# qpc001/ORB_SLAM2_Commit

Measured on AMD Instinct MI355X. Metric: frames/sec ORB extract+match (2k kp) + LocalBA iters/sec, KITTI-00 stereo, higher is better.
Workload: dtype u8; 1 GPU; KITTI-00 stereo 1241x376, 2000 features, extract L+R + ComputeStereoMatches; batch_frames_per_gpu=256, global_batch_frames=256, nlevels=8, parallelism=frame-sharded x1, batches_in_flight=4

## Files before the change

include/orbx_debug.h:

```cpp
#ifndef ORBX_DEBUG_H
#define ORBX_DEBUG_H
#include "orbx.h"
#ifdef __cplusplus
extern "C" {
#endif

enum {
  ORBX_DBG_BLUR_LEVEL = 1,
  ORBX_DBG_CELL_COUNTS = 2,
  ORBX_DBG_CELL_TABLE = 3,
  ORBX_DBG_CANDIDATES = 4,
  ORBX_DBG_OCT_COUNTS = 5,
  ORBX_DBG_OCT_OUT = 6,
  ORBX_DBG_LEVEL_INFO = 7,
  ORBX_DBG_PATCH_SLOTS = 8
};

long long orbx_debug_copy(orbx_extractor* h, int what, int image, int arg, void* dst, size_t cap);

enum {
  ORBX_LP_LEVELS = 1,
  ORBX_LP_RESIZE = 2,
  ORBX_LP_BOUNDS = 3,
  ORBX_LP_GRIDS = 4,
  ORBX_LP_REMAP = 5,
  ORBX_LP_XTAB = 6,
  ORBX_LP_YTAB = 7,
  ORBX_LP_PATH = 8,
  ORBX_LP_FAST = 9,
  ORBX_LP_OCTREE = 10,
  ORBX_LP_CELLS = 11,
  ORBX_LP_OCT_LEVELS = 12,
  ORBX_LP_OCT_PYRAMID = 13
};
long long orbx_debug_launch_plan(const orbx_extractor_params* params, int width, int height, int what, int a0,
                                 int a1, int a2, long long* dst, size_t cap);

orbx_status orbx_debug_stereo_keypoints(orbx_extractor* left, orbx_extractor* right, const orbx_keypoint* kpsL,
                                        const uint8_t* descL, int nL, const orbx_keypoint* kpsR, const uint8_t* descR,
                                        int nR, float bf, float baseline, float* uRight, float* depth, int32_t* sad,
                                        int32_t* nmatches);
int orbx_debug_stereo_keypoints_check(const orbx_keypoint* kps, int n, int nlevels, int width, int height);

orbx_status orbx_debug_octree_candidates(orbx_extractor* h, int n_img, const int32_t* cell_counts,
                                         const uint32_t* candidates, int32_t* oct_count, uint32_t* oct_out);
orbx_status orbx_debug_octree_paths(orbx_extractor* h, int n_img, const int32_t* cell_counts,
                                    const uint32_t* candidates, int depth_cap, int32_t* oct_count,
                                    uint32_t* oct_out, int32_t* paths);
int orbx_debug_octree_candidates_check(const orbx_extractor_params* params, int width, int height, int n_img,
                                       const int32_t* cell_counts, const uint32_t* candidates);

double orbx_debug_atan2_det(double y, double x);

int orbx_debug_lm_step(double state[5], int counts[2], double tempChi, double scale, int ok2, int cube_kind,
                       int ops);

int orbx_debug_exp(const double* x, int n, double* y, int device);
int orbx_debug_sim3_exp(const double update[7], const double S[8], int fix_scale, double out[8], int device);

int orbx_debug_log(const double* x, int n, double* y, int device);
int orbx_debug_acos(const double* x, int n, double* y, int device);
int orbx_debug_sim3_log(const double* S, int n, double* out, int32_t* branch, int device);
int orbx_debug_essgraph_linearize(const orbx_essential_graph_problem* problem, double* meas, double* err,
                                  double* J0, double* J1, double* H, double* b, int device);
int orbx_debug_essgraph_solve(const orbx_essential_graph_problem* problem, const double* H, const double* b,
                              double lambda, double* x, int32_t* ok, int device);
int orbx_debug_essgraph_phases(const orbx_essential_graph_problem* problem, const orbx_essential_graph_result* result,
                               double phase_ms[3], long long* envelope_blocks, int device);

int orbx_debug_ldlt(const double* S, const double* b, int N, double* x, int reps, float* ms);
int orbx_debug_ldlt_ex(const double* S, const double* b, int N, double* x, int reps, float* ms, int kind,
                       unsigned long long* stamps);

#define ORBX_BA_LDLT_AUTO 0
#define ORBX_BA_LDLT_COLUMN 1
#define ORBX_BA_LDLT_BLOCKED 2
#define ORBX_BA_LDLT_TILED 3
typedef struct {
  int ldlt;
  int nan_trial;
  int raise_stop_after;
  int trace;
  int fused_ctl;
} orbx_ba_debug_options;
int orbx_debug_ba_options(orbx_ba* h, const orbx_ba_debug_options* options);

enum {
  ORBX_BA_CAP_HEADER = 0,
  ORBX_BA_CAP_LAMBDA_CHI = 1,
  ORBX_BA_CAP_CQ = 2,
  ORBX_BA_CAP_CT = 3,
  ORBX_BA_CAP_X = 4,
  ORBX_BA_CAP_EERR = 5,
  ORBX_BA_CAP_S = 6,
  ORBX_BA_CAP_BS = 7,
  ORBX_BA_CAP_XP = 8,
  ORBX_BA_CAP_CBAK = 9,
  ORBX_BA_CAP_XBAK = 10,
  ORBX_BA_CAP_XL = 11,
  ORBX_BA_CAP_ACT = 12,
  ORBX_BA_CAP_POSE_CAM = 13,
  ORBX_BA_CAP_PT_ID = 14,
  ORBX_BA_CAP_EROBUST = 15
};
int orbx_debug_ba_capture_select(orbx_ba* h, int phase, int it, int q);
long long orbx_debug_ba_capture_read(orbx_ba* h, int what, void* dst, size_t cap);

int orbx_debug_hbm_copy(void* dst, const void* src, size_t bytes, int reps, float* ms);

int orbx_debug_initializer_host(const float* keys1_xy, int n1, const float K[9], float sigma, int iterations,
                                const float* keys2_xy, int n2, const int32_t* matches12, const int32_t* rand_vals,
                                int n_rand, int* used, float R21[9], float t21[3], float* p3d,
                                uint8_t* triangulated, orbx_initializer_result* result);
float orbx_debug_acosf_det(float x);

typedef struct {
  int raise_after_neighbour;
  int probes;
} orbx_new_points_debug_options;
int orbx_debug_new_points_options(orbx_new_points* h, const orbx_new_points_debug_options* options);
enum {
  ORBX_NP_PROBE_EXIT = 0,
  ORBX_NP_PROBE_COS = 1,
  ORBX_NP_PROBE_F12 = 2,
  ORBX_NP_PROBE_MATCH12 = 3
};
long long orbx_debug_new_points_probe(orbx_new_points* h, int what, void* dst, size_t cap);
int orbx_debug_new_points_host(const orbx_new_points_problem* problem, int neighbour, const int32_t* match12,
                               int32_t* skip, float* baseline, float* median_depth, float F12[9], uint8_t* exit_code,
                               float* cos3, float* pos, float* normal, float* dist);

#ifdef __cplusplus
}
#endif
#endif
```

orb_slam2_commit_amd/_lib.py:

```python
import ctypes as C
import os

import numpy as np

_HERE = os.path.dirname(os.path.abspath(__file__))
LIB_PATH = os.environ.get("ORBX_LIB_OVERRIDE") or os.path.join(_HERE, "liborbx.so")

ORBX_OK = 0
ORBX_ERR_ARG = -1
ORBX_ERR_CAPACITY = -2
ORBX_ERR_HIP = -3
ORBX_ERR_NODEV = -4
ORBX_ERR_SIZE = -5
ORBX_ERR_STATE = -6
ORBX_DEPTH_U16 = 2
ORBX_DEPTH_F32 = 5
_ERRS = {ORBX_ERR_ARG: "bad argument", ORBX_ERR_CAPACITY: "capacity", ORBX_ERR_HIP: "HIP runtime error",
         ORBX_ERR_NODEV: "no HIP device", ORBX_ERR_SIZE: "unsupported geometry", ORBX_ERR_STATE: "no extraction yet"}

KEYPOINT_DTYPE = np.dtype([("x", "<f4"), ("y", "<f4"), ("size", "<f4"), ("angle", "<f4"),
                           ("response", "<f4"), ("octave", "<i4"), ("class_id", "<i4")])
assert KEYPOINT_DTYPE.itemsize == 28


# ... 212 lines not shown
    "orbx_extractor_get_levels": ([P], C.c_int),
    "orbx_extractor_scale_tables": ([P, P, P, P, P], C.c_int),
    "orbx_extractor_tables": ([P, P, P, P], C.c_int),
    "orbx_extractor_set_pyramid_readback": ([P, C.c_int], C.c_int),
    "orbx_extractor_max_keypoints": ([P, C.c_int, C.c_int], C.c_int),
    "orbx_extract": ([P, P, C.c_int, C.c_int, C.c_size_t, P, C.c_int, P, C.POINTER(C.c_int)], C.c_int),
    "orbx_pyramid_level": ([P, C.c_int, C.c_int, P, C.c_size_t, C.POINTER(C.c_int), C.POINTER(C.c_int)], C.c_int),
    "orbx_extract_batch_device": ([P, C.c_int, P, C.c_int, C.c_int, C.c_size_t, P, P, P, C.c_int, P], C.c_int),
    "orbx_stereo_match": ([P, P, P, P, C.c_int, P, P, C.c_int, C.c_float, C.c_float, P, P], C.c_int),
    "orbx_frame_stereo": ([P, P, C.c_size_t, P, C.c_size_t, C.c_int, C.c_int, C.c_float, C.c_float, P, P, C.c_int, P,
                           P, P, C.c_int, P, P, P], C.c_int),
    "orbx_stereo_frames_device": ([P, C.c_int, P, C.c_int, C.c_int, C.c_size_t, P, P, P, C.c_int, C.c_float,
                                   C.c_float, P, P, P, P], C.c_int),
    "orbx_cvt_gray": ([P, C.c_size_t, C.c_size_t, C.c_int, C.c_int, C.c_int, C.c_int, C.c_int, P, C.c_size_t,
                       C.c_size_t, C.c_int], C.c_int),
    "orbx_cvt_gray_device": ([P, P, C.c_size_t, C.c_size_t, C.c_int, C.c_int, C.c_int, C.c_int, C.c_int, P,
                              C.c_size_t, C.c_size_t, P], C.c_int),
    "orbx_frame_rgbd": ([P, P, C.c_size_t, C.c_int, C.c_int, C.c_int, C.c_int, P, C.c_size_t, C.c_int, C.c_int,
                         C.c_int, C.c_float, C.POINTER(Camera), C.c_float, P, P, C.c_int, C.POINTER(C.c_int), P, P,
                         P], C.c_int),
    "orbx_rgbd_frames_device": ([P, C.c_int, P, C.c_int, C.c_int, C.c_int, C.c_int, C.c_size_t, C.c_size_t, P,
                                 C.c_int, C.c_size_t, C.c_size_t, C.c_float, C.POINTER(Camera), C.c_float, P, P, P,
                                 C.c_int, P, P, P, P, P], C.c_int),
    "orbx_descriptor_distance_device": ([P, P, C.c_int, P, P], C.c_int),
    "orbx_search_by_bow_kf_f": ([C.POINTER(BowSide), C.POINTER(BowSide), C.c_float, C.c_int, P,
                                 C.POINTER(C.c_int), C.c_int], C.c_int),
    "orbx_search_by_bow_kf_kf": ([C.POINTER(BowSide), C.POINTER(BowSide), C.c_float, C.c_int, P,
                                  C.POINTER(C.c_int), C.c_int], C.c_int),
    "orbx_search_by_bow_device": ([C.POINTER(BowProblem), C.c_int, P], C.c_int),
    "orbx_pnp_create": ([C.POINTER(PnpProblem), C.POINTER(PnpParams), C.c_int, C.POINTER(C.c_void_p)], C.c_int),
    "orbx_pnp_create_many": ([P, C.c_int, C.POINTER(PnpParams), C.c_int, P], C.c_int),
    "orbx_pnp_create_many_device": ([P, P, P, P, P, C.c_int, C.POINTER(PnpParams), C.c_int, P], C.c_int),
    "orbx_pnp_destroy": ([P], C.c_int),
    "orbx_pnp_get_params": ([P, C.POINTER(C.c_int), C.POINTER(C.c_int), C.POINTER(C.c_float)], C.c_int),
    "orbx_pnp_set_ransac_parameters": ([P, P, C.POINTER(PnpParams)], C.c_int),
    "orbx_pnp_iterate": ([P, C.c_int, P, C.c_int, C.POINTER(C.c_int), C.POINTER(C.c_int), P, P,
                          C.POINTER(C.c_int), C.POINTER(C.c_int)], C.c_int),
    "orbx_pnp_iterate_stream": ([P, C.c_int, C.POINTER(RandState), C.POINTER(C.c_int), P, P, C.POINTER(C.c_int),
                                 C.POINTER(C.c_int)], C.c_int),
    "orbx_voc_load_text": ([C.c_char_p, C.c_size_t, C.c_int, C.POINTER(C.c_void_p)], C.c_int),
    "orbx_voc_destroy": ([P], C.c_int),
    "orbx_voc_info": ([P, P], C.c_int),
    "orbx_voc_transform": ([P, P, P, C.c_int, C.c_int, P, P, P, P, P, P, P], C.c_int),
    "orbx_voc_transform_device": ([P, P, C.c_int, C.c_longlong, P, C.c_int, C.c_int, C.c_int, P, P, P, P, P, P, P, P],
                                  C.c_int),
    "orbx_kfdb_create": ([P, C.c_int, C.POINTER(C.c_void_p)], C.c_int),
    "orbx_kfdb_destroy": ([P], C.c_int),
    "orbx_kfdb_check_bow": ([P, P, C.c_int, C.c_uint32], C.c_int),
    "orbx_kfdb_add": ([P, C.c_int64, P, P, C.c_int], C.c_int),
    "orbx_kfdb_erase": ([P, C.c_int64], C.c_int),
    "orbx_kfdb_clear": ([P], C.c_int),
    "orbx_kfdb_set_neighbours": ([P, P, P, P, C.c_int], C.c_int),
    "orbx_kfdb_reloc_candidates": ([P, C.c_uint64, P, P, C.c_int, P, C.c_int, C.POINTER(C.c_int)], C.c_int),
    "orbx_kfdb_loop_candidates": ([P, C.c_uint64, P, P, C.c_int, P, C.c_int, C.c_float, P, C.c_int,
                                   C.POINTER(C.c_int)], C.c_int),
    "orbx_kfdb_reloc_candidates_device": ([P, C.c_uint64, P, P, P, P, C.c_int, P, P], C.c_int),
    "orbx_kfdb_loop_candidates_device": ([P, C.c_uint64, P, P, P, P, C.c_int, C.c_float, P, C.c_int, P, P],
                                         C.c_int),
    "orbx_kfdb_score": ([P, P, P, C.c_int, P, C.c_int, P], C.c_int),
    "orbx_kfdb_read_state": ([P, P, C.c_int, P, P, P, P, P, P], C.c_int),
    "orbx_kfdb_size": ([P, C.POINTER(C.c_int), C.POINTER(C.c_longlong)], C.c_int),
    "orbx_covis_create": ([C.c_int, C.POINTER(C.c_void_p)], C.c_int),
    "orbx_covis_destroy": ([P], C.c_int),
    "orbx_covis_clear": ([P], C.c_int),
    "orbx_covis_check_row": ([P, P, P, C.c_int], C.c_int),
    "orbx_covis_set_keyframe": ([P, C.c_int64, C.c_int, P, P, P], C.c_int),
    "orbx_covis_erase_keyframe": ([P, C.c_int64], C.c_int),
    "orbx_covis_set_points_bad": ([P, P, C.c_int], C.c_int),
    "orbx_covis_size": ([P, C.POINTER(C.c_int), C.POINTER(C.c_longlong), C.POINTER(C.c_int)], C.c_int),
    "orbx_covis_read_keyframe": ([P, C.c_int64, P, P, P, C.c_int, C.POINTER(C.c_int)], C.c_int),
    "orbx_covis_read_points": ([P, P, C.c_int, P, P], C.c_int),
    "orbx_covis_update_connections": ([P, C.c_int64, C.c_int, P, P, C.c_int, C.POINTER(C.c_int), P, P, C.c_int,
                                       C.POINTER(C.c_int)], C.c_int),
    "orbx_covis_vote": ([P, P, C.c_int, P, P, P, C.c_int, C.POINTER(C.c_int), C.POINTER(C.c_int64),
                         C.POINTER(C.c_int32)], C.c_int),
    "orbx_covis_local_points": ([P, P, C.c_int, P, C.c_int, C.POINTER(C.c_int)], C.c_int),
    "orbx_covis_cull": ([P, P, C.c_int, P, C.c_int, P, P, C.c_int, C.POINTER(C.c_int)], C.c_int),
    "orbx_track_gather_device": ([C.POINTER(TrackGather), C.c_int, P], C.c_int),
    "orbx_frame_points_device": ([C.POINTER(FramePoints), C.c_int, P], C.c_int),
    "orbx_track_step_device": ([C.POINTER(TrackStep), C.c_int, P], C.c_int),
    "orbx_search_by_projection": ([C.POINTER(ProjProblem), C.c_int], C.c_int),
    "orbx_search_by_sim3": ([C.POINTER(Sim3Problem), C.c_int], C.c_int),
    "orbx_search_for_initialization": ([C.POINTER(InitProblem), C.c_int], C.c_int),
    "orbx_search_by_projection_device": ([C.POINTER(ProjProblem), C.c_int, P], C.c_int),
    "orbx_pose_optimization": ([C.POINTER(PoseProblem), C.c_int], C.c_int),
    "orbx_pose_optimization_device": ([C.POINTER(PoseProblem), C.c_int, P], C.c_int),
    "orbx_optimize_sim3": ([C.POINTER(OptSim3Problem), C.c_int], C.c_int),
    "orbx_optimize_sim3_device": ([C.POINTER(OptSim3Problem), C.c_int, P], C.c_int),
    "orbx_optimize_essential_graph": ([C.POINTER(EssGraphProblem), C.POINTER(EssGraphResult), C.c_int], C.c_int),
    "orbx_optimize_essential_graph_device": ([C.POINTER(EssGraphProblem), C.POINTER(EssGraphResult), P], C.c_int),
    "orbx_sim3_from_tcw": ([P, P], None),
    "orbx_search_for_triangulation": ([C.POINTER(TriProblem), C.c_int], C.c_int),
    "orbx_search_for_triangulation_device": ([C.POINTER(TriProblem), C.c_int, P], C.c_int),
    "orbx_new_points_create": ([C.c_int, C.POINTER(C.c_void_p)], C.c_int),
    "orbx_new_points_destroy": ([P], C.c_int),
    "orbx_new_points_stop_flag": ([P, C.POINTER(C.POINTER(C.c_int))], C.c_int),
    "orbx_create_new_map_points": ([P, C.POINTER(NewPointsProblem), C.POINTER(NewPointsResult)], C.c_int),
    "orbx_create_new_map_points_bool": ([P, C.POINTER(NewPointsProblem), C.POINTER(NewPointsResult), P], C.c_int),
    "orbx_create_new_map_points_device": ([P, C.POINTER(NewPointsProblem), C.POINTER(NewPointsResult), P], C.c_int),
    "orbx_distinctive_descriptors": ([P, P, C.c_int, P, P, C.c_int], C.c_int),
    "orbx_distinctive_descriptors_device": ([P, P, C.c_int, P, P, P], C.c_int),
    "orbx_undistort_keypoints": ([P, C.c_int, C.POINTER(Camera), P, C.c_int], C.c_int),
    "orbx_undistort_keypoints_device": ([P, P, C.c_int, C.c_int, P, P, P], C.c_int),
    "orbx_pnp_iterate_candidates": ([P, C.c_int, C.c_int, C.POINTER(RandState), P, P, C.POINTER(C.c_int)], C.c_int),
    "orbx_pnp_iterate_many": ([P, C.c_int, C.c_int, P, P, P], C.c_int),
    "orbx_sim3_create": ([C.POINTER(Sim3SolverProblem), C.POINTER(Sim3Params), C.c_int, C.POINTER(C.c_void_p)],
                         C.c_int),
    "orbx_sim3_create_many": ([P, C.c_int, C.POINTER(Sim3Params), C.c_int, P], C.c_int),
    "orbx_sim3_destroy": ([P], C.c_int),
    "orbx_sim3_set_ransac_parameters": ([P, C.POINTER(Sim3Params)], C.c_int),
    "orbx_sim3_get_params": ([P, C.POINTER(C.c_int), C.POINTER(C.c_int), C.POINTER(C.c_int), C.POINTER(C.c_int)],
                             C.c_int),
    "orbx_sim3_iterate": ([P, C.c_int, P, C.c_int, C.POINTER(C.c_int), C.POINTER(C.c_int), P, P,
                           C.POINTER(C.c_int), C.POINTER(C.c_int)], C.c_int),
    "orbx_sim3_iterate_stream": ([P, C.c_int, C.POINTER(RandState), C.POINTER(C.c_int), P, P, C.POINTER(C.c_int),
                                  C.POINTER(C.c_int)], C.c_int),
    "orbx_sim3_get_estimate": ([P, P, P, C.POINTER(C.c_float)], C.c_int),
    "orbx_sim3_iterate_candidates": ([P, C.c_int, C.c_int, C.POINTER(RandState), P, P, C.POINTER(C.c_int)],
                                     C.c_int),
    "orbx_sim3_iterate_many": ([P, C.c_int, C.c_int, P, P, P], C.c_int),
    "orbx_initializer_create": ([P, C.c_int, P, C.c_float, C.c_int, C.c_int, C.POINTER(C.c_void_p)], C.c_int),
    "orbx_initializer_destroy": ([P], C.c_int),
    "orbx_initializer_initialize": ([P, P, C.c_int, P, P, C.c_int, C.POINTER(C.c_int), P, P, P, P,
                                     C.POINTER(InitializerResult)], C.c_int),
    "orbx_initializer_initialize_stream": ([P, P, C.c_int, P, C.POINTER(RandState), P, P, P, P,
                                            C.POINTER(InitializerResult)], C.c_int),
    "orbx_rand_seed":([C.POINTER(RandState), C.c_uint32], None),
    "orbx_rand_next": ([C.POINTER(RandState)], C.c_int32),
    "orbx_ba_create": ([C.c_int, C.POINTER(C.c_void_p)], C.c_int),
    "orbx_ba_create_priority": ([C.c_int, C.c_int, C.POINTER(C.c_void_p)], C.c_int),
    "orbx_ba_create_masked": ([C.c_int, C.c_void_p, C.c_int, C.POINTER(C.c_void_p)], C.c_int),
    "orbx_stream_create": ([C.c_int, C.c_void_p, C.c_int, C.POINTER(C.c_void_p)], C.c_int),
    "orbx_stream_destroy": ([C.c_void_p], None),
    "orbx_ba_destroy": ([P], C.c_int),
    "orbx_ba_run": ([P, C.POINTER(BaProblem), C.POINTER(BaResult), P], C.c_int),
    "orbx_ba_run_bool": ([P, C.POINTER(BaProblem), C.POINTER(BaResult), P], C.c_int),
    "orbx_ba_run_global": ([P, C.POINTER(BaProblem), C.c_int, C.c_int, C.POINTER(BaResult), P, P], C.c_int),
    "orbx_ba_run_global_bool": ([P, C.POINTER(BaProblem), C.c_int, C.c_int, C.POINTER(BaResult), P, P], C.c_int),
    "orbx_ba_stop_flag":([P, C.POINTER(C.POINTER(C.c_int))], C.c_int),
    "orbx_ba_run_many": ([P, C.c_int, C.POINTER(BaProblem), C.POINTER(BaResult), P], C.c_int),
    "orbx_local_ba": ([C.POINTER(BaProblem), C.POINTER(BaResult), P, C.c_int], C.c_int),
    "orbx_device_count": ([], C.c_int),
    "orbx_version": ([], C.c_char_p),
    "orbx_sizeof": ([C.c_char_p], C.c_longlong),
    "orbx_profile_enable": ([P, C.c_int], C.c_int),
    "orbx_profile_reset": ([P], C.c_int),
    "orbx_profile_read": ([P, C.c_int, C.POINTER(C.c_double), C.POINTER(C.c_longlong),
                           C.POINTER(C.c_char_p)], C.c_int),
    "orbx_debug_copy": ([P, C.c_int, C.c_int, C.c_int, P, C.c_size_t], C.c_longlong),
    "orbx_debug_launch_plan": ([C.POINTER(ExtractorParams), C.c_int, C.c_int, C.c_int, C.c_int, C.c_int, C.c_int, P,
                                C.c_size_t], C.c_longlong),
    "orbx_debug_stereo_keypoints": ([P, P, P, P, C.c_int, P, P, C.c_int, C.c_float, C.c_float, P, P, P, P], C.c_int),
    "orbx_debug_stereo_keypoints_check": ([P, C.c_int, C.c_int, C.c_int, C.c_int], C.c_int),
    "orbx_debug_octree_candidates": ([P, C.c_int, P, P, P, P], C.c_int),
    "orbx_debug_octree_paths": ([P, C.c_int, P, P, C.c_int, P, P, P], C.c_int),    "orbx_debug_octree_candidates_check": ([C.POINTER(ExtractorParams), C.c_int, C.c_int, C.c_int, P, P], C.c_int),
    "orbx_debug_atan2_det": ([C.c_double, C.c_double], C.c_double),
    "orbx_debug_exp": ([P, C.c_int, P, C.c_int], C.c_int),
    "orbx_debug_initializer_host": ([P, C.c_int, P, C.c_float, C.c_int, P, C.c_int, P, P, C.c_int,
                                     C.POINTER(C.c_int), P, P, P, P, C.POINTER(InitializerResult)], C.c_int),
    "orbx_debug_acosf_det": ([C.c_float], C.c_float),
    "orbx_debug_lm_step": ([P, P, C.c_double, C.c_double, C.c_int, C.c_int, C.c_int], C.c_int),
    "orbx_debug_sim3_exp": ([P, P, C.c_int, P, C.c_int], C.c_int),
    "orbx_debug_log": ([P, C.c_int, P, C.c_int], C.c_int),
    "orbx_debug_acos": ([P, C.c_int, P, C.c_int], C.c_int),
    "orbx_debug_sim3_log": ([P, C.c_int, P, P, C.c_int], C.c_int),
    "orbx_debug_essgraph_linearize": ([C.POINTER(EssGraphProblem), P, P, P, P, P, P, C.c_int], C.c_int),
    "orbx_debug_essgraph_solve": ([C.POINTER(EssGraphProblem), P, P, C.c_double, P, P, C.c_int], C.c_int),
    "orbx_debug_essgraph_phases": ([C.POINTER(EssGraphProblem), C.POINTER(EssGraphResult), P, P, C.c_int], C.c_int),
    "orbx_debug_ldlt": ([P, P, C.c_int, P, C.c_int, C.POINTER(C.c_float)], C.c_int),
    "orbx_debug_ldlt_ex": ([P, P, C.c_int, P, C.c_int, C.POINTER(C.c_float), C.c_int, P], C.c_int),
    "orbx_debug_ba_options": ([P, C.POINTER(BaDebugOptions)], C.c_int),
    "orbx_debug_ba_capture_select": ([P, C.c_int, C.c_int, C.c_int], C.c_int),
    "orbx_debug_ba_capture_read": ([P, C.c_int, P, C.c_size_t], C.c_longlong),
    "orbx_debug_new_points_options": ([P, C.POINTER(NewPointsDebugOptions)], C.c_int),
    "orbx_debug_new_points_probe": ([P, C.c_int, P, C.c_size_t], C.c_longlong),
    "orbx_debug_new_points_host": ([C.POINTER(NewPointsProblem), C.c_int, P, P, P, P, P, P, P, P, P, P], C.c_int),
    "orbx_debug_hbm_copy": ([P, P, C.c_size_t, C.c_int, C.POINTER(C.c_float)], C.c_int),
}

BA_CAPTURE_ITEMS = {
    "lambda_chi": (1, np.float64, ()), "cq": (2, np.float64, (4,)), "ct": (3, np.float64, (3,)),
    "X": (4, np.float64, (3,)), "eerr": (5, np.float64, (3,)), "S": (6, np.float64, ()), "bs": (7, np.float64, ()),
    "xp": (8, np.float64, ()), "cbak": (9, np.float64, (7,)), "Xbak": (10, np.float64, (3,)),
    "xl": (11, np.float64, (3,)), "act": (12, np.int32, ()), "pose_cam": (13, np.int32, ()),
    "pt_id": (14, np.int32, ()), "erobust": (15, np.int32, ()),
}
BA_CAPTURE_HEADER = ("fired", "phase", "it", "q", "ok", "trial", "nc", "np", "ne", "na", "npa", "nposes")

_lib = None
_NEWER_ENTRIES = {"orbx_debug_octree_paths"}


def lib():
    global _lib
    if _lib is None:
        if not os.path.exists(LIB_PATH):
            raise RuntimeError("liborbx.so not found at %s -- build it first (make -C orb_slam2_commit_amd/csrc)"
                               % LIB_PATH)
        L = C.CDLL(LIB_PATH)
        for name, (args, res) in SIGNATURES.items():
            if name in _NEWER_ENTRIES and os.environ.get("ORBX_LIB_OVERRIDE") and not hasattr(L, name):
                continue
            fn = getattr(L, name)
            fn.argtypes = args
            fn.restype = res
        _lib = L
    return _lib


def check(code, what):
    if code != ORBX_OK:
        raise OrbxError(code, what)


def ptr(a):
    if a is None:
        return None
    if isinstance(a, np.ndarray):
        try:
            return C.c_void_p(C.addressof(C.c_char.from_buffer(a)))
        except (TypeError, ValueError, BufferError):
            return C.c_void_p(a.__array_interface__["data"][0])
    if hasattr(a, "data_ptr"):
        return C.c_void_p(a.data_ptr())
    raise TypeError(type(a))
```

orb_slam2_commit_amd/csrc/capi.hip:

```cpp
#include <hip/hip_runtime.h>

#include <cmath>
#include <new>
#include <string>

#include "orbx_extractor.h"
#include "orbx_rgbd.h"
#include "orbx_undistort.h"

namespace orbx {

orbx_status get_plan(orbx_extractor* h, int W, int H, DevPlan** out) {
  auto key = std::make_pair(W, H);
  auto it = h->plans.find(key);
  if (it != h->plans.end()) {
    *out = it->second.get();
    return ORBX_OK;
  }
  std::unique_ptr<DevPlan> P(new (std::nothrow) DevPlan());
  if (!P) return ORBX_ERR_HIP;
  orbx_status s = build_plan(h->params, h->tables, W, H, *P);
  if (s != ORBX_OK) return s;
  hipError_t e = P->dG.upload(&P->G, 1);
  if (e == hipSuccess) e = P->dcells.upload(P->cells.data(), P->cells.size());
  if (e == hipSuccess) e = P->dtiles.upload(P->tile_level.data(), P->tile_level.size());
  if (e == hipSuccess) e = P->drzb.upload(P->rzb.data(), P->rzb.size());
  if (e == hipSuccess) e = P->dxt.upload(P->xt.data(), P->xt.size());
  if (e == hipSuccess) e = P->dyt.upload(P->yt.data(), P->yt.size());
  if (e != hipSuccess) return ORBX_ERR_HIP;
  build_launch_plan(*P, P->dxt.p, P->dyt.p, P->drzb.p, P->LP);
  size_t mx = octree_group_smem(P->G.og_all);
  for (int g = 0; g < P->G.n_og; g++) mx = std::max(mx, octree_group_smem(P->G.og[g]));
  if (octree_set_smem_limit(mx) != hipSuccess) return ORBX_ERR_HIP;
  *out = P.get();
  h->plans[key] = std::move(P);
  return ORBX_OK;
}

orbx_status ensure_batch(orbx_extractor* h, const Plan& P, int n) {
  const Geometry& G = P.G;
  hipError_t e = hipSuccess;
  auto chk = [&](hipError_t x) { if (x != hipSuccess) e = x; };
  chk(h->pyr.ensure((size_t)G.pyr_bytes * n + 256));
  chk(h->blur.ensure((size_t)G.blur_bytes * n + 256));
  chk(h->cand.ensure((size_t)G.cand_total * n));
  chk(h->kpos.ensure((size_t)G.cand_total * n));
  chk(h->knode.ensure((size_t)G.cand_total * n));
  chk(h->cell_count.ensure((size_t)std::max(G.ncells, 1) * n));
  chk(h->oct.ensure((size_t)G.oct_total * n));
  chk(h->oct_count.ensure((size_t)G.nlevels * n));
  return hip_status(e);
}

BatchPtrs batch_ptrs(orbx_extractor* h, const uint8_t* in, size_t pitch) {
  BatchPtrs B;
  B.in = in;
  B.in_pitch = pitch;
  B.pyr = h->pyr.p;
  B.blur = h->blur.p;
  B.cand = h->cand.p;
  B.cell_count = h->cell_count.p;
  B.kpos = h->kpos.p;
  B.knode = h->knode.p;
  B.oct = h->oct.p;
  B.oct_count = h->oct_count.p;
  return B;
}

orbx_status run_extract(orbx_extractor* h, DevPlan* P, int n, const uint8_t* d_in, size_t pitch, orbx_keypoint* d_kps,
                        uint8_t* d_desc, int32_t* d_counts, int kp_cap, hipStream_t st) {
  if (kp_cap < P->G.max_kps) return ORBX_ERR_CAPACITY;
  orbx_status s = ensure_batch(h, *P, n);
  if (s != ORBX_OK) return s;
  BatchPtrs B = batch_ptrs(h, d_in, pitch);
  hipError_t e = launch_extract_stages(P->G, P->dG.p, P->dcells.p, P->dtiles.p, P->LP, B, n, d_kps, d_desc, d_counts, kp_cap, st,
                                       &h->timer);
  if (e != hipSuccess) return ORBX_ERR_HIP;
  h->last_plan = P;
  h->last_in = d_in;
  h->last_pitch = pitch;
  h->last_n = n;
  h->last_host = false;
  h->hpyr_valid = false;
  return ORBX_OK;
}

orbx_status run_stereo(orbx_extractor* hl, orbx_extractor* hr, int n_frames, const StereoSides& S, int maxL, float bf,
                       float baseline, float* uR, float* depth, long long out_stride, int32_t* nmatches,
                       hipStream_t st) {
  orbx_extractor* h = hl;
  const DevPlan* P = hl->last_plan;
  hipError_t e = hipSuccess;
  auto chk = [&](hipError_t x) { if (x != hipSuccess) e = x; };
  chk(h->rkeys.ensure((size_t)n_frames * kMaxStereoKps));
  chk(h->oct_start.ensure((size_t)n_frames * (kMaxLevelsPlan + 1)));
  chk(h->rxi.ensure((size_t)n_frames * kMaxStereoKps));
  chk(h->rdesc.ensure((size_t)n_frames * kMaxStereoKps * 2));
  chk(h->rtab.ensure((size_t)n_frames * P->G.nlevels * std::max(P->G.height, 1)));
  chk(h->lrange.ensure((size_t)n_frames * std::max(maxL, 1)));
  chk(h->sad.ensure((size_t)n_frames * out_stride));
  if (e != hipSuccess) return ORBX_ERR_HIP;
  StereoArgs A;
  std::memset(&A, 0, sizeof(A));
  A.kpL = S.L.kps;
  A.dL = S.L.desc;
  A.nL = S.L.counts;
  A.kL_stride = S.L.k_stride;
  A.n_stride_L = S.L.n_stride;
  A.l_step = S.L.step;
  A.l_off = S.L.off;
  A.kpR = S.R.kps;
  A.dR = S.R.desc;
  A.nR = S.R.counts;
  A.kR_stride = S.R.k_stride;
  A.n_stride_R = S.R.n_stride;
  A.r_step = S.R.step;
  A.r_off = S.R.off;
  A.BL = batch_ptrs(hl, hl->last_in, hl->last_pitch);
  A.BR = batch_ptrs(hr, hr->last_in, hr->last_pitch);
  A.nlevels = P->G.nlevels;
  A.maxL = maxL;
  for (int l = 0; l < P->G.nlevels; l++) A.inv_scale[l] = hl->tables.inv_scale[l];
  A.bf = bf;
  A.minZ = baseline;
  A.minD = 0.f;
  A.maxD = bf / baseline;
  A.uR = uR;
  A.depth = depth;
  A.sad = h->sad.p;
  A.out_stride = out_stride;
  A.rkeys = h->rkeys.p;
  A.oct_start = h->oct_start.p;
  A.rxi = h->rxi.p;
  A.rdesc = h->rdesc.p;
  A.rtab = h->rtab.p;
  A.lrange = h->lrange.p;
  A.rows = std::max(P->G.height, 1);
  A.nmatches = nmatches;
  return hip_status(launch_stereo(A, P->dG.p, n_frames, maxL, st, &h->timer));
}

}

using namespace orbx;

namespace {

constexpr size_t kInSlack = 4;

uint64_t fingerprint_words(const void* p, size_t nw, uint64_t h) {
  const uint32_t* w = reinterpret_cast<const uint32_t*>(p);
  for (size_t i = 0; i < nw; i++) {
    h = (h ^ w[i]) * 0x9E3779B97F4A7C15ull;
    h ^= h >> 29;
  }
  return h;
}
uint64_t keypoint_fingerprint(const orbx_keypoint* k, const uint8_t* desc, int n) {
  uint64_t h = 1469598103934665603ull ^ (uint64_t)n;
  h = fingerprint_words(k, (size_t)n * (sizeof(orbx_keypoint) / 4), h);
  if (desc) h = fingerprint_words(desc, (size_t)n * 8, h ^ 0xD6E8FEB86659FD93ull);
  return h;
}


}

extern "C" {

const char* orbx_version(void) { return "orbx 0.1.0 (gfx950)"; }

long long orbx_sizeof(const char* type) {
  if (!type) return -1;
  const std::string t(type);
#define ORBX_SIZEOF(T) \
  if (t == #T) return (long long)sizeof(T);
  ORBX_SIZEOF(orbx_keypoint) ORBX_SIZEOF(orbx_extractor_params) ORBX_SIZEOF(orbx_bow_side)
  ORBX_SIZEOF(orbx_bow_problem) ORBX_SIZEOF(orbx_ba_problem) ORBX_SIZEOF(orbx_ba_result)
  ORBX_SIZEOF(orbx_pnp_problem) ORBX_SIZEOF(orbx_pnp_params) ORBX_SIZEOF(orbx_pnp_result)
  ORBX_SIZEOF(orbx_rand_state) ORBX_SIZEOF(orbx_proj_frame) ORBX_SIZEOF(orbx_proj_problem)
  ORBX_SIZEOF(orbx_tri_kf) ORBX_SIZEOF(orbx_tri_problem) ORBX_SIZEOF(orbx_pose_problem)
  ORBX_SIZEOF(orbx_track_gather) ORBX_SIZEOF(orbx_frame_points) ORBX_SIZEOF(orbx_track_step)
  ORBX_SIZEOF(orbx_camera) ORBX_SIZEOF(orbx_sim3_problem) ORBX_SIZEOF(orbx_init_problem)
  ORBX_SIZEOF(orbx_sim3_solver_problem) ORBX_SIZEOF(orbx_sim3_params) ORBX_SIZEOF(orbx_sim3_result)
  ORBX_SIZEOF(orbx_optimize_sim3_problem) ORBX_SIZEOF(orbx_essential_graph_problem)
  ORBX_SIZEOF(orbx_essential_graph_result) ORBX_SIZEOF(orbx_new_points_kf)
  ORBX_SIZEOF(orbx_new_points_problem) ORBX_SIZEOF(orbx_new_points_result)
#undef ORBX_SIZEOF
  return -1;
}

int orbx_device_count(void) {
  int n = 0;
  if (hipGetDeviceCount(&n) != hipSuccess) return 0;
  return n;
}

orbx_status orbx_extractor_create(const orbx_extractor_params* params, int device, orbx_extractor** out) {
  if (!out || !params_ok(params)) return ORBX_ERR_ARG;
  *out = nullptr;
  int n = 0;
  if (hipGetDeviceCount(&n) != hipSuccess || n <= 0) return ORBX_ERR_NODEV;
  if (device < 0 || device >= n) return ORBX_ERR_ARG;
  if (hipSetDevice(device) != hipSuccess) return ORBX_ERR_HIP;
  orbx_extractor* h = new (std::nothrow) orbx_extractor();
  if (!h) return ORBX_ERR_HIP;
  h->params = *params;
  h->device = device;
  h->tables = make_tables(*params);
  int gauss[7];
  gaussian_int_kernel(gauss);
  if (upload_constants(h->tables.umax, gauss) != hipSuccess ||
      hipStreamCreateWithFlags(&h->stream, hipStreamNonBlocking) != hipSuccess) {
    delete h;
    return ORBX_ERR_HIP;
  }
  *out = h;
  return ORBX_OK;
}

void orbx_extractor_destroy(orbx_extractor* h) {
  if (!h) return;
  (void)hipSetDevice(h->device);
  if (h->stream) {
    (void)hipStreamSynchronize(h->stream);
    (void)hipStreamDestroy(h->stream);
  }
  delete h;
}

int orbx_extractor_get_levels(const orbx_extractor* h) { return h ? h->params.nlevels : ORBX_ERR_ARG; }

orbx_status orbx_extractor_scale_tables(const orbx_extractor* h, float* scale, float* inv_scale, float* sigma2,
                                        float* inv_sigma2) {
  if (!h) return ORBX_ERR_ARG;
  const int n = h->params.nlevels;
  for (int i = 0; i < n; i++) {
    if (scale) scale[i] = h->tables.scale[i];
    if (inv_scale) inv_scale[i] = h->tables.inv_scale[i];
    if (sigma2) sigma2[i] = h->tables.sigma2[i];
    if (inv_sigma2) inv_sigma2[i] = h->tables.inv_sigma2[i];
  }
  return ORBX_OK;
}

orbx_status orbx_extractor_tables(const orbx_extractor* h, int* features_per_level, int* umax, int* pattern) {
  if (!h) return ORBX_ERR_ARG;
  static const int8_t kPattern[512 * 2] = {
#include "brief_pattern_31.inc"
  };
  for (int i = 0; i < h->params.nlevels; i++)
    if (features_per_level) features_per_level[i] = h->tables.nfeat[i];
  for (int v = 0; v < 16; v++)
    if (umax) umax[v] = h->tables.umax[v];
  for (int i = 0; i < 1024; i++)
    if (pattern) pattern[i] = kPattern[i];
  return ORBX_OK;
}

orbx_status orbx_extractor_set_pyramid_readback(orbx_extractor* h, int on) {
  if (!h) return ORBX_ERR_ARG;
  h->pyr_readback = on != 0;
  if (!h->pyr_readback) h->hpyr_valid = false;
  return ORBX_OK;
}

int orbx_extractor_max_keypoints(orbx_extractor* h, int width, int height) {
  if (!h) return ORBX_ERR_ARG;
  DevPlan* P = nullptr;
  orbx_status s = get_plan(h, width, height, &P);
  return s == ORBX_OK ? P->G.max_kps : s;
}

orbx_status orbx_extract(orbx_extractor* h, const uint8_t* img, int width, int height, size_t stride,
                         orbx_keypoint* kps, int cap, uint8_t* desc, int* n) {
  if (!h || !n) return ORBX_ERR_ARG;
  *n = 0;
  if (!img || width <= 0 || height <= 0) return ORBX_OK;
  if (stride < (size_t)width) return ORBX_ERR_ARG;
  if (hipSetDevice(h->device) != hipSuccess) return ORBX_ERR_HIP;
  DevPlan* P = nullptr;
  orbx_status s = get_plan(h, width, height, &P);
  if (s != ORBX_OK) return s;
  const int kcap = P->G.max_kps;
// ... 463 lines not shown
```

orb_slam2_commit_amd/csrc/debug.hip:

```cpp
#include <hip/hip_runtime.h>

#include <cmath>
#include <vector>

#include "../../include/orbx_debug.h"
#include "orbx_extractor.h"

using namespace orbx;

extern "C" long long orbx_debug_copy(orbx_extractor* h, int what, int image, int arg, void* dst, size_t cap) {
  if (!h) return ORBX_ERR_ARG;
  if (!h->last_plan) return ORBX_ERR_STATE;
  const DevPlan& P = *h->last_plan;
  const Geometry& G = P.G;
  if (image < 0 || image >= h->last_n) return ORBX_ERR_ARG;
  if (hipSetDevice(h->device) != hipSuccess) return ORBX_ERR_HIP;
  if (hipStreamSynchronize(h->stream) != hipSuccess) return ORBX_ERR_HIP;
  std::vector<int> host;
  const void* src = nullptr;
  size_t bytes = 0;
  bool device_src = true;
  switch (what) {
    case ORBX_DBG_BLUR_LEVEL: {
      if (arg < 0 || arg >= G.nlevels) return ORBX_ERR_ARG;
      const LevelGeom& L = G.lv[arg];
      bytes = (size_t)L.w * L.h;
      if (dst && cap >= bytes) {
        if (h->blur.ensure((size_t)G.blur_bytes * h->last_n + 256) != hipSuccess) return ORBX_ERR_HIP;
        const BatchPtrs B = batch_ptrs(h, h->last_in, h->last_pitch);
        if (launch_blur(G, P.dG.p, P.dtiles.p, B, h->last_n, h->stream) != hipSuccess ||
            hipStreamSynchronize(h->stream) != hipSuccess)
          return ORBX_ERR_HIP;
        const uint8_t* b = h->blur.p + (size_t)image * G.blur_bytes + L.boff;
        std::vector<uint8_t> tiles((size_t)L.bstride * ((L.h + 7) & ~7));
        if (hipMemcpy(tiles.data(), b, tiles.size(), hipMemcpyDeviceToHost) != hipSuccess) return ORBX_ERR_HIP;
        uint8_t* o = static_cast<uint8_t*>(dst);
        for (int yy = 0; yy < L.h; yy++)
          for (int xx = 0; xx < L.w; xx++)
            o[(size_t)yy * L.w + xx] = tiles[((size_t)(yy >> 3) * (L.bstride >> 4) + (xx >> 4)) * 128 + (yy & 7) * 16 + (xx & 15)];
      }
      return (long long)bytes;
    }
    case ORBX_DBG_CELL_COUNTS:
      src = h->cell_count.p + (size_t)image * G.ncells;
      bytes = sizeof(int) * G.ncells;
      break;
    case ORBX_DBG_CELL_TABLE: {
      int loff = 0;
      for (const CellInfo& c : P.cells) {
        int v[8] = {c.level, c.x0, c.y0, c.x1, c.y1, loff, c.cap, 0};
        host.insert(host.end(), v, v + 8);
        loff += c.cap;
      }
      device_src = false;
      break;
    }
    case ORBX_DBG_CANDIDATES: {
      std::vector<uint32_t> raw((size_t)G.cand_total);
      if (hipMemcpy(raw.data(), h->cand.p + (size_t)image * G.cand_total, raw.size() * 4, hipMemcpyDeviceToHost) !=
          hipSuccess)
        return ORBX_ERR_HIP;
      std::vector<uint32_t> logical;
      logical.reserve(raw.size());
      for (const CellInfo& c : P.cells)
        for (int q = 0; q < c.cap; q++) logical.push_back(raw[cell_slot(c, q)]);
      static_assert(sizeof(uint32_t) == sizeof(int), "host staging is int words");
      host.resize(logical.size());
      std::memcpy(host.data(), logical.data(), logical.size() * 4);
      device_src = false;
      break;
    }
    case ORBX_DBG_OCT_COUNTS:
      src = h->oct_count.p + (size_t)image * G.nlevels;
      bytes = sizeof(int) * G.nlevels;
      break;
    case ORBX_DBG_OCT_OUT:
      src = h->oct.p + (size_t)image * G.oct_total;
      bytes = sizeof(uint32_t) * G.oct_total;
      break;
    case ORBX_DBG_LEVEL_INFO:
      for (int l = 0; l < G.nlevels; l++) {
        const LevelGeom& L = G.lv[l];
        int v[8] = {L.w, L.h, L.cell_begin, L.cell_end, L.oct_off, L.oct_cap, L.nfeat, L.nIni};
        host.insert(host.end(), v, v + 8);
      }
      device_src = false;
      break;
    case ORBX_DBG_PATCH_SLOTS:
      host.assign(patch_slot_table(), patch_slot_table() + 128);
      device_src = false;
      break;
    default:
      return ORBX_ERR_ARG;
  }
  if (!device_src) {
    bytes = host.size() * sizeof(int);
    if (dst) std::memcpy(dst, host.data(), std::min(bytes, cap));
    return (long long)bytes;
  }
  if (dst && cap) {
    if (hipMemcpy(dst, src, std::min(bytes, cap), hipMemcpyDeviceToHost) != hipSuccess) return ORBX_ERR_HIP;
  }
  return (long long)bytes;
}

extern "C" int orbx_debug_stereo_keypoints_check(const orbx_keypoint* kps, int n, int nlevels, int width,
                                                 int height) {
  if (n < 0 || (n > 0 && !kps) || nlevels < 1 || nlevels > kMaxLevelsPlan || width <= 0 || height <= 0)
    return ORBX_ERR_ARG;
  for (int i = 0; i < n; i++) {
    const orbx_keypoint& k = kps[i];
    if (k.octave < 0 || k.octave >= nlevels) return ORBX_ERR_ARG;
    if (!std::isfinite(k.x) || !std::isfinite(k.y) || std::signbit(k.x) || std::signbit(k.y)) return ORBX_ERR_ARG;
    if (!(k.x < (float)width) || !(k.y < (float)height)) return ORBX_ERR_ARG;
  }
  return ORBX_OK;
}

extern "C" orbx_status orbx_debug_stereo_keypoints(orbx_extractor* left, orbx_extractor* right,
                                                   const orbx_keypoint* kpsL, const uint8_t* descL, int nL,
                                                   const orbx_keypoint* kpsR, const uint8_t* descR, int nR, float bf,
                                                   float baseline, float* uRight, float* depth, int32_t* sad,
                                                   int32_t* nmatches) {
  if (!uRight || !depth || !sad || !nmatches || nL < 0 || nR < 0) return ORBX_ERR_ARG;
  if ((nL > 0 && (!kpsL || !descL)) || (nR > 0 && (!kpsR || !descR))) return ORBX_ERR_ARG;
  if (nR > kMaxStereoKps) return ORBX_ERR_CAPACITY;
  if (!left || !right) return ORBX_ERR_ARG;
  if (!left->last_plan || !right->last_plan || !left->last_host || !right->last_host) return ORBX_ERR_STATE;
  const Geometry& G = left->last_plan->G;
  if (G.width != right->last_plan->G.width || G.height != right->last_plan->G.height ||
      G.nlevels != right->last_plan->G.nlevels || left->device != right->device)
    return ORBX_ERR_ARG;
  if (orbx_debug_stereo_keypoints_check(kpsL, nL, G.nlevels, G.width, G.height) != ORBX_OK ||
      orbx_debug_stereo_keypoints_check(kpsR, nR, G.nlevels, G.width, G.height) != ORBX_OK)
    return ORBX_ERR_ARG;
  *nmatches = 0;
  if (nL == 0) return ORBX_OK;
  orbx_extractor* h = left;
  if (hipSetDevice(h->device) != hipSuccess) return ORBX_ERR_HIP;
  BlockCursor cur;
  const size_t o_kL = cur.take<orbx_keypoint>(nL), o_kR = cur.take<orbx_keypoint>(nR),
               o_dL = cur.take<uint8_t>((size_t)nL * 32), o_dR = cur.take<uint8_t>((size_t)nR * 32),
               o_res = cur.take<float>((size_t)2 * nL);
  DevBuf<uint8_t> blk;
  if (blk.ensure(cur.end()) != hipSuccess) return ORBX_ERR_HIP;
  hipError_t e = hipSuccess;
  auto chk = [&](hipError_t x) { if (x != hipSuccess) e = x; };
  hipStream_t st = h->stream;
  const int32_t counts[3] = {nL, nR, 0};
  chk(hipMemcpyAsync(blk.p, counts, sizeof(counts), hipMemcpyHostToDevice, st));
  chk(hipMemcpyAsync(blk.p + o_kL, kpsL, (size_t)nL * sizeof(orbx_keypoint), hipMemcpyHostToDevice, st));
  chk(hipMemcpyAsync(blk.p + o_dL, descL, (size_t)nL * 32, hipMemcpyHostToDevice, st));
  if (nR > 0) {
    chk(hipMemcpyAsync(blk.p + o_kR, kpsR, (size_t)nR * sizeof(orbx_keypoint), hipMemcpyHostToDevice, st));
    chk(hipMemcpyAsync(blk.p + o_dR, descR, (size_t)nR * 32, hipMemcpyHostToDevice, st));
  }
  if (e != hipSuccess) {
    (void)hipStreamSynchronize(st);
    return ORBX_ERR_HIP;
  }
  int32_t* d_counts = (int32_t*)blk.p;
  float* d_ur = (float*)(blk.p + o_res);
  const StereoSides S = StereoSides::handles((const orbx_keypoint*)(blk.p + o_kL), blk.p + o_dL, d_counts,
                                             (const orbx_keypoint*)(blk.p + o_kR), blk.p + o_dR, d_counts + 1);
  orbx_status s = run_stereo(left, right, 1, S, nL, bf, baseline, d_ur, d_ur + nL, nL, d_counts + 2, st);
  if (s == ORBX_OK) {
    chk(hipMemcpyAsync(uRight, d_ur, sizeof(float) * nL, hipMemcpyDeviceToHost, st));
    chk(hipMemcpyAsync(depth, d_ur + nL, sizeof(float) * nL, hipMemcpyDeviceToHost, st));
    chk(hipMemcpyAsync(sad, h->sad.p, sizeof(int32_t) * nL, hipMemcpyDeviceToHost, st));
    chk(hipMemcpyAsync(nmatches, d_counts + 2, sizeof(int32_t), hipMemcpyDeviceToHost, st));
  }
  chk(hipStreamSynchronize(st));
  if (s != ORBX_OK) return s;
  return hip_status(e);
}

constexpr int kOctInjectMaxImages = 64;
static bool octree_candidates_ok(const Plan& P, int n_img, const int32_t* counts, const uint32_t* cand) {
  const Geometry& G = P.G;
  if (n_img < 1 || n_img > kOctInjectMaxImages || !counts || !cand || G.ncells < 1) return false;
  long long total = 0;
  for (const CellInfo& c : P.cells) total += c.cap;
  std::vector<uint8_t> seen;
  for (int img = 0; img < n_img; img++) {
    const int32_t* cnt = counts + (size_t)img * G.ncells;
    const uint32_t* cd = cand + (size_t)img * total;
    for (int l = 0; l < G.nlevels; l++) {
      const LevelGeom& L = G.lv[l];
      seen.assign((size_t)L.w * L.h, 0);
      for (int ci = L.cell_begin; ci < L.cell_end; ci++) {
        if (cnt[ci] < 0 || cnt[ci] > P.cells[ci].cap) return false;
        for (int q = 0; q < cnt[ci]; q++) {
          const uint32_t v = cd[q];
          const int x = (int)(v & 0xFFF), y = (int)((v >> 12) & 0xFFF);
          if (x < L.minBX || x >= L.maxBX || y < L.minBY || y >= L.maxBY) return false;
          uint8_t& s = seen[(size_t)y * L.w + x];
          if (s) return false;
          s = 1;
        }
        cd += P.cells[ci].cap;
      }
    }
  }
  return true;
}

extern "C" int orbx_debug_octree_candidates_check(const orbx_extractor_params* params, int width, int height,
                                                  int n_img, const int32_t* cell_counts, const uint32_t* candidates) {
  if (!params_ok(params) || width <= 0 || height <= 0) return ORBX_ERR_ARG;
  Plan P;
  const orbx_status s = build_plan(*params, make_tables(*params), width, height, P);
  if (s != ORBX_OK) return s;
  return octree_candidates_ok(P, n_img, cell_counts, candidates) ? ORBX_OK : ORBX_ERR_ARG;
}

static orbx_status octree_candidates_run(orbx_extractor* h, int n_img, const int32_t* cell_counts,
                                         const uint32_t* candidates, int32_t* oct_count, uint32_t* oct_out,
                                         int32_t* paths, int depth_cap) {
  if (!h || !oct_count || !oct_out) return ORBX_ERR_ARG;
  if (!h->last_plan) return ORBX_ERR_STATE;
  const DevPlan& P = *h->last_plan;
  const Geometry& G = P.G;
  if (!octree_candidates_ok(P, n_img, cell_counts, candidates)) return ORBX_ERR_ARG;
  if (hipSetDevice(h->device) != hipSuccess) return ORBX_ERR_HIP;
  const size_t n = (size_t)n_img;
  BlockCursor cur;
  const size_t o_cand = cur.take<uint32_t>(n * G.cand_total), o_cnt = cur.take<int>(n * G.ncells),
               o_kpos = cur.take<uint32_t>(n * G.cand_total), o_knode = cur.take<int>(n * G.cand_total),
               o_oct = cur.take<uint32_t>(n * G.oct_total), o_octn = cur.take<int>(n * G.nlevels),
               o_path = cur.take<int>(n * G.nlevels);
  DevBuf<uint8_t> blk;
  if (blk.ensure(cur.end()) != hipSuccess) return ORBX_ERR_HIP;
  std::vector<uint32_t> raw(n * G.cand_total, 0);
  {
    const uint32_t* cd = candidates;
    for (int img = 0; img < n_img; img++)
      for (int ci = 0; ci < G.ncells; ci++) {
        const CellInfo& c = P.cells[ci];
        for (int q = 0; q < cell_counts[(size_t)img * G.ncells + ci]; q++)
          raw[(size_t)img * G.cand_total + cell_slot(c, q)] = cd[q];
        cd += c.cap;
      }
  }
  hipError_t e = hipSuccess;
  auto chk = [&](hipError_t x) { if (x != hipSuccess) e = x; };
  hipStream_t st = h->stream;
  chk(hipMemcpyAsync(blk.p + o_cand, raw.data(), raw.size() * 4, hipMemcpyHostToDevice, st));
  chk(hipMemcpyAsync(blk.p + o_cnt, cell_counts, n * G.ncells * sizeof(int), hipMemcpyHostToDevice, st));
  chk(hipMemsetAsync(blk.p + o_oct, 0xFF, n * G.oct_total * 4, st));
  chk(hipMemsetAsync(blk.p + o_octn, 0xFF, n * G.nlevels * sizeof(int), st));
  chk(hipMemsetAsync(blk.p + o_path, 0xFF, n * G.nlevels * sizeof(int), st));
  if (e == hipSuccess) {
    BatchPtrs B{};
    B.cand = (uint32_t*)(blk.p + o_cand);
    B.cell_count = (int*)(blk.p + o_cnt);
    B.kpos = (uint32_t*)(blk.p + o_kpos);
    B.knode = (int*)(blk.p + o_knode);
    B.oct = (uint32_t*)(blk.p + o_oct);
    B.oct_count = (int*)(blk.p + o_octn);
    size_t mx = octree_group_smem(G.og_all);
    for (int g = 0; g < G.n_og; g++) mx = std::max(mx, octree_group_smem(G.og[g]));
    chk(octree_set_smem_limit(mx));
    if (e == hipSuccess)
      chk(launch_octree(G, P.dG.p, P.dcells.p, B, n_img, st, paths ? (int*)(blk.p + o_path) : nullptr, depth_cap));
  }
  if (e == hipSuccess && paths)
    chk(hipMemcpyAsync(paths, blk.p + o_path, n * G.nlevels * sizeof(int), hipMemcpyDeviceToHost, st));
  if (e == hipSuccess) {
    chk(hipMemcpyAsync(oct_count, blk.p + o_octn, n * G.nlevels * sizeof(int), hipMemcpyDeviceToHost, st));
    chk(hipMemcpyAsync(oct_out, blk.p + o_oct, n * G.oct_total * 4, hipMemcpyDeviceToHost, st));
  }
  chk(hipStreamSynchronize(st));
  return hip_status(e);
}

extern "C" orbx_status orbx_debug_octree_candidates(orbx_extractor* h, int n_img, const int32_t* cell_counts,
                                                    const uint32_t* candidates, int32_t* oct_count,
                                                    uint32_t* oct_out) {
  return octree_candidates_run(h, n_img, cell_counts, candidates, oct_count, oct_out, nullptr, -1);
}

extern "C" orbx_status orbx_debug_octree_paths(orbx_extractor* h, int n_img, const int32_t* cell_counts,
                                               const uint32_t* candidates, int depth_cap, int32_t* oct_count,
                                               uint32_t* oct_out, int32_t* paths) {
  if (!paths || depth_cap < -1) return ORBX_ERR_ARG;
  return octree_candidates_run(h, n_img, cell_counts, candidates, oct_count, oct_out, paths, depth_cap);
}

extern "C" long long orbx_debug_launch_plan(const orbx_extractor_params* params, int width, int height, int what,
                                            int a0, int a1, int a2, long long* dst, size_t cap) {
  std::vector<long long> out;
  auto done = [&]() {
    if (dst) std::memcpy(dst, out.data(), std::min(out.size(), cap) * sizeof(long long));
    return (long long)out.size();
  };
  if (what == ORBX_LP_REMAP) {
    XcdRemap R{};
    if (a0 < 1 || a1 < 1 || a2 < 1 || !make_xcd_remap((unsigned)a0, (unsigned)a1, (unsigned)a2, &R)) return ORBX_ERR_ARG;
    out = {R.gx, R.gy, R.q, R.r, R.mx, R.sx, R.my, R.sy};
    return done();
  }
  if (!params_ok(params) || width <= 0 || height <= 0) return ORBX_ERR_ARG;
  Plan P;
  const orbx_status s = build_plan(*params, make_tables(*params), width, height, P);
  if (s != ORBX_OK) return s;
  LaunchPlan LP;
  build_launch_plan(P, P.xt.data(), P.yt.data(), P.rzb.data(), LP);
  const Geometry& G = P.G;
  switch (what) {
    case ORBX_LP_LEVELS:
      for (int l = 0; l < G.nlevels; l++) {
        const LevelGeom& L = G.lv[l];
        out.insert(out.end(), {L.w, L.h, L.off, L.boff, L.bstride, L.tile_begin, L.tiles_x, L.tiles_y});
      }
      break;
    case ORBX_LP_RESIZE:
      for (int l = 1; l < G.nlevels; l++) {
        const ResizeDesc& D = LP.rz[l];
        out.insert(out.end(), {D.sw, D.sh, D.dw, D.dh, D.src_off, D.dst_off, D.pyr_bytes, D.X - P.xt.data(),
                               D.Y - P.yt.data(), D.bx - P.rzb.data(), D.by - P.rzb.data(), D.stride, D.rows, D.lc,
                               (D.dw + kRzTW - 1) / kRzTW, (D.dh + kRzTH - 1) / kRzTH});
      }
      break;
    case ORBX_LP_BOUNDS:
      for (int i = 0; i < P.rzb_n; i++) out.insert(out.end(), {P.rzb[i].x, P.rzb[i].y});
      break;
    case ORBX_LP_PATH:
      for (int l = 1; l < G.nlevels; l++) {
        const bool f = P.strip[l];
// ... 106 lines not shown
```

orb_slam2_commit_amd/csrc/extract.hip:

```cpp
#include <hip/hip_runtime.h>

#include <utility>

#include "orbx_device.h"
#include "orbx_internal.h"
#include "orbx_prof.h"

namespace orbx {

__constant__ float c_pattern_f[1024] = {
#include "brief_pattern_31.inc"
};
__constant__ uint4 c_icmask[64];
__constant__ double c_sincos[23] = {
    6.36619772367581382433e-01,
    1.57079632673412561417e+00,
    6.07710050650619224932e-11,
    1.0 / 51090942171709440000.0, -1.0 / 121645100408832000.0, 1.0 / 355687428096000.0,
    -1.0 / 1307674368000.0,       1.0 / 6227020800.0,           -1.0 / 39916800.0,
    1.0 / 362880.0,               -1.0 / 5040.0,                1.0 / 120.0,
    -1.0 / 6.0,
    1.0 / 2432902008176640000.0,  -1.0 / 6402373705728000.0,    1.0 / 20922789888000.0,
    -1.0 / 87178291200.0,         1.0 / 479001600.0,            -1.0 / 3628800.0,
    1.0 / 40320.0,                -1.0 / 720.0,                 1.0 / 24.0,
// ... 773 lines not shown
    return max(max(max(n0, n1), max(n2, n3)), max(max(n4, n5), max(n6, n7)));
  };
  auto kept = [](int s, int mx, int thr) -> bool {
    return s >= max(mx + 1, max(thr, 2));
  };
  auto keep = [&](int e, int thr) -> bool { return kept(smap[e + S + 1], ring8_max(e), thr); };
  FAST_TS(1);
  int nc = detect(ini);
  FAST_TS(2);
#ifdef ORBX_FAST_PROBE
  n_corner_ini = nc;
#endif
  int cnt = 0;
  for (int i0 = 0; i0 < nc; i0 += 64) {
    const int i = i0 + lane;
    int e = 0, s = 0, mx = 0;
    if (i < nc) {
      e = list[i];
      s = smap[e + S + 1];
      mx = ring8_max(e);
    }
    const bool k = kept(s, mx, ini + 1);
    const uint64_t km = ballot64(k);
    if (k) list[i] = (uint16_t)(e | 0x8000);
    cnt += __popcll(km);
  }
  FAST_TS(3);
  if (cnt == 0 && mint != ini) nc = detect(mint);
  FAST_TS(4);
  const int thr = (cnt > 0 ? ini : mint) + 1;
  uint32_t* const out = B.cand + (size_t)img * G->cand_total + c.ovf_off - c.kin;
  uint32_t* const out_in = B.cand + (size_t)img * G->cand_total + c.cand_off;
  const int kin = c.kin;
  int pos = 0;
  for (int i0 = 0; i0 < nc; i0 += 64) {
    const int i = i0 + lane;
    int e = 0;
    bool k = false;
    if (i < nc) {
      const int le = list[i];
      e = le & 0x7FFF;
      k = cnt > 0 ? (le >> 15) != 0 : keep(e, thr);
    }
    const uint64_t m = __ballot(k);
    if (k) {
      const int p = pos + lane_rank(m);
      const int y = e / S, x = e - y * S;
      if (p < c.cap)
      {
        const uint32_t v = ((uint32_t)(smap[e + S + 1] - 1) << 24) | ((uint32_t)(c.y0 + y) << 12) | (uint32_t)(c.x0 + x);
        if (p < kin) out_in[p]= v; else out[p] = v;
      }
    }
    pos += __popcll(m);
  }
  if (lane == 0) B.cell_count[(size_t)img * G->ncells + cell] = min(pos, c.cap);
#ifdef ORBX_FAST_PROBE
  FAST_TS(5);
  if (lane < 8 && fast_probe_buf) {
    const unsigned long long t[8] = {ts1 - ts0, ts_mid - ts1, ts2 - ts_mid, ts3 - ts2, ts4 - ts3, ts5 - ts4,
                                     (unsigned long long)((cnt == 0) | (n_corner_ini << 1) | (cnt << 16)),
                                     (unsigned long long)(n_compass | (n_even8 << 16))};
    fast_probe_buf[((size_t)img * G->ncells + cell) * 8 + lane] = (unsigned int)t[lane];
  }
#endif
  }
}

template <int S, int RP, int N0>
static auto fast_kernel(int nk) -> decltype(&k_fast<S, RP, N0>) {
  return nk <= N0 ? k_fast<S, RP, N0> : k_fast<S, RP, N0 + 1>;
}

struct OctSmem {
  int16_t* x0;
  int16_t* y0;
  int16_t* x1;
  int16_t* y1;
  int* cnt;
  int* seq;
  int* ccnt;
  int16_t* cidx;
  int16_t* nidx;
  int* sa;
  int* sb;
  uint64_t* key;
  int* cpre;
  int* ctrl;
  uint32_t* kp;
  uint16_t* kn;
};

constexpr int kOctRankSortMax = 1024;

template <int NT>
__device__ __forceinline__ void bitonic_sort_desc(uint64_t* k, int n) {
  for (int size = 2; size <= n; size <<= 1) {
    for (int stride = size >> 1; stride > 0; stride >>= 1) {
      for (int i = threadIdx.x; i < n / 2; i += NT) {
        const int lo = 2 * i - (i & (stride - 1));
        const int hi = lo + stride;
        const bool desc = (lo & size) == 0;
        const uint64_t a = k[lo], b = k[hi];
        if (desc ? (a < b) : (a > b)) {
          k[lo] = b;
          k[hi] = a;
        }
      }
      __syncthreads();
    }
  }
}

struct OctCands {
  uint32_t* lpos;
  uint16_t* lnd;
  int kcap;
  uint32_t* gpos;
  uint32_t* gnd;
  __device__ __forceinline__ uint32_t pos(int k) const { return k < kcap ? lpos[k] : gpos[k]; }
  __device__ __forceinline__ uint32_t nd(int k) const { return k < kcap ? (uint32_t)lnd[k] : gnd[k]; }
  __device__ __forceinline__ void set(int k, uint32_t p, uint32_t n) const {
    if (k < kcap) {
      lpos[k] = p;
      lnd[k] = (uint16_t)n;
    } else {
      gpos[k] = p;
      gnd[k] = n;
    }
  }
  __device__ __forceinline__ void set_nd(int k, uint32_t n) const {
    if (k < kcap) lnd[k] = (uint16_t)n; else gnd[k] = n;
  }
};

template <int NT, class F>
__device__ __forceinline__ void oct_cands(int T, const OctCands& c, F f) {
  for (int k = threadIdx.x; k < T; k += NT) {
    const uint32_t n0 = c.nd(k);
    uint32_t n = n0;
    f(k, c.pos(k), n);
    if (n != n0) c.set_nd(k, n);
  }
}

#ifdef ORBX_OCT_PROBE
constexpr int kOctProbeWords = 12;
__device__ unsigned int* oct_probe_buf;
#define OCT_TS(v) const unsigned long long v = __builtin_amdgcn_s_memtime()
#else
#define OCT_TS(v)
#endif

template <int NT>
__device__ int oct_generic(const Geometry* __restrict__ G, const CellInfo* __restrict__ cells, const BatchPtrs& B,
                           const OctGroup& grp, unsigned char* smem_raw, int img, int l) {
  const int tid = threadIdx.x;
  const LevelGeom& L = G->lv[l];
  const int NC = grp.node_cap;
  const int NP2 = next_pow2(NC);
  OctSmem s;
  {
    unsigned char* p = smem_raw;
    s.x0 = (int16_t*)p; p += NC * 4;
    s.y0 = (int16_t*)p; p += NC * 4;
    s.x1 = (int16_t*)p; p += NC * 4;
    s.y1 = (int16_t*)p; p += NC * 4;
    s.cnt = (int*)p; p += NC * 8;
    s.seq = (int*)p; p += NC * 8;
    s.ccnt = (int*)p; p += NC * 16;
    s.cidx = (int16_t*)p; p += NC * 8;
    s.nidx = (int16_t*)p; p += NC * 2;
    s.sa = (int*)p; p += NC * 4;
    s.sb = (int*)p; p += NC * 4;
    p = (unsigned char*)(((uintptr_t)p + 7) & ~(uintptr_t)7);
    s.key = (uint64_t*)p; p += (size_t)NP2 * 8;
    s.cpre = (int*)p; p += (grp.cell_cap + 1) * 4;
    s.ctrl = (int*)p; p += 8 * 4;
    s.kp = (uint32_t*)p; p += (size_t)grp.kcap * 4;
    s.kn = (uint16_t*)p;
  }
  uint32_t* oct_out = B.oct + (size_t)img * G->oct_total + L.oct_off;
  int* oct_cnt = B.oct_count + (size_t)img * G->nlevels + l;
  const size_t kbase = (size_t)img * G->cand_total + L.cand_begin;
  OctCands oc{s.kp, s.kn, grp.kcap, B.kpos + kbase, (uint32_t*)B.knode + kbase};

  OCT_TS(ot0);
#ifdef ORBX_OCT_PROBE
  unsigned long long ot_p1 = 0, ot_p2 = 0;
  int n_p1 = 0, n_p2 = 0;
#endif
  const int ncl = L.cell_end - L.cell_begin;
  for (int c = tid; c < ncl; c += NT) s.cpre[c] = B.cell_count[(size_t)img * G->ncells + L.cell_begin + c];
  __syncthreads();
  const int T = block_exclusive_scan<NT>(s.cpre, ncl);
  if (tid == 0) s.cpre[ncl] = T;
  if (T == 0) {
    if (tid == 0) *oct_cnt = 0;
    return 0;
  }
  const int nIni = L.nIni;
  const float hX = L.hX;
  const int minBX = L.minBX, minBY = L.minBY;
  for (int i = tid; i < nIni; i += NT) s.ccnt[i] = 0;
  __syncthreads();
  const uint32_t* cand = B.cand + (size_t)img * G->cand_total;
  auto put_cand = [&](int k, uint32_t v) {
    const int xr = (int)(v & 0xFFF) - minBX, yr = (int)((v >> 12) & 0xFFF) - minBY;
    const uint32_t pos = (v & 0xFF000000u) | ((uint32_t)yr << 12) | (uint32_t)xr;
    int root = (int)((float)xr / hX);
    root = min(max(root, 0), nIni - 1);
    oc.set(k, pos, (uint32_t)root);
    atomicAdd(&s.ccnt[root], 1);
  };
  if (ncl >= NT / 2) {
    for (int c = tid; c < ncl; c += NT) {
      const int k0 = s.cpre[c], n = s.cpre[c + 1] - k0;
      const CellInfo& ci = cells[L.cell_begin + c];
      const int kin = ci.kin, off = ci.cand_off, ovf = ci.ovf_off - kin;
      int i = 0;
      for (; i + 4 <= n; i += 4) {
        const uint32_t v0 = cand[(i < kin ? off : ovf) + i], v1 = cand[(i + 1 < kin ? off : ovf) + i + 1],
                       v2 = cand[(i + 2 < kin ? off : ovf) + i + 2], v3 = cand[(i + 3 < kin ? off : ovf) + i + 3];
        put_cand(k0 + i, v0);
        put_cand(k0 + i + 1, v1);
        put_cand(k0 + i + 2, v2);
        put_cand(k0 + i + 3, v3);
      }
      for (; i < n; i++) put_cand(k0 + i, cand[(i < kin ? off : ovf) + i]);
    }
  } else {
    for (int k = tid; k < T; k += NT) {
      int lo = 0, hi = ncl - 1;
      while (lo < hi) {
        const int mid = (lo + hi + 1) >> 1;
        if (s.cpre[mid] <= k) lo = mid; else hi = mid - 1;
      }
      put_cand(k, cand[cell_slot(cells[L.cell_begin + lo], k - s.cpre[lo])]);
    }
  }
  __syncthreads();
  OCT_TS(ot1);
  for (int i = tid; i < nIni; i += NT) s.sa[i] = s.ccnt[i] > 0 ? 1 : 0;
  __syncthreads();
  int S = block_exclusive_scan<NT>(s.sa, nIni);
  for (int i = tid; i < nIni; i += NT) {
    if (s.ccnt[i] > 0) {
      const int ni = s.sa[i];
      s.x0[ni] = (int16_t)(int)(hX * (float)i);
      s.x1[ni] = (int16_t)(int)(hX * (float)(i + 1));
      s.y0[ni] = 0;
      s.y1[ni] = (int16_t)(L.maxBY - minBY);
      s.cnt[ni] = s.ccnt[i];
      s.seq[ni] = i;
      s.nidx[i] = (int16_t)ni;
    }
  }
  __syncthreads();
  oct_cands<NT>(T, oc, [&](int, uint32_t, uint32_t& nd) { nd = (uint32_t)s.nidx[nd]; });
  for (int i = tid; i < S * 4; i += NT) s.ccnt[i] = 0;
  OCT_TS(ot2);
  int cur = 0;
  int seqBase = nIni;
  int phase = 1;
  const int N = L.nfeat;
  for (int round = 0; round < 256; round++) {
    __syncthreads();
#ifdef ORBX_OCT_PROBE
    const unsigned long long rt0 = __builtin_amdgcn_s_memtime();
    const int rphase = phase;
    struct RoundStamp {
      unsigned long long t0;
      int ph;
      unsigned long long *p1, *p2;
      int *n1, *n2;
      __device__ ~RoundStamp() {
        const unsigned long long d = __builtin_amdgcn_s_memtime() - t0;
        if (ph == 1) { *p1 += d; ++*n1; } else { *p2 += d; ++*n2; }
      }
    } rstamp{rt0, rphase, &ot_p1, &ot_p2, &n_p1, &n_p2};
#endif
    const int nb = cur ^ 1;
    oct_cands<NT>(T, oc, [&](int, uint32_t v, uint32_t& nd) {
      const int n = (int)(nd & 0x3FFF);
      if ((s.cnt + cur * NC)[n] > 1) {
        const int nx0 = (s.x0 + cur * NC)[n], ny0 = (s.y0 + cur * NC)[n];
        const int hx = (int)__builtin_ceilf((float)((s.x1 + cur * NC)[n] - nx0) / 2);
        const int hy = (int)__builtin_ceilf((float)((s.y1 + cur * NC)[n] - ny0) / 2);
        const float fx = (float)(int)(v & 0xFFF), fy = (float)(int)((v >> 12) & 0xFFF);
        const int d = (fx < (float)(nx0 + hx) ? 0 : 1) + (fy < (float)(ny0 + hy) ? 0 : 2);
        nd = (uint32_t)n | ((uint32_t)d << 14);
        atomicAdd(&s.ccnt[n * 4 + d], 1);
      }
    });
    __syncthreads();
    int C, Snew;
    if (phase == 1) {
      for (int i = tid; i < S; i += NT) {
        const bool split = (s.cnt + cur * NC)[i] > 1;
        uint64_t v = split ? 0 : (1ull << 16);
        if (split)
          for (int d = 0; d < 4; d++) {
            const int cc = s.ccnt[i * 4 + d];
            v += (cc > 0 ? 1ull : 0ull) + (cc > 1 ? (1ull << 32) : 0ull);
          }
        s.key[i] = v;
      }
      __syncthreads();
      const uint64_t tot = block_scan_excl<NT, uint64_t>(s.key, S);
      C = (int)(tot & 0xFFFF);
      const int Sg = (int)((tot >> 16) & 0xFFFF);
      const int nexp = (int)(tot >> 32);
      for (int i = tid; i < S; i += NT) {
        const uint64_t pre = s.key[i];
        if ((s.cnt + cur * NC)[i] > 1) {
          const int nx0 = (s.x0 + cur * NC)[i], ny0 = (s.y0 + cur * NC)[i], nx1 = (s.x1 + cur * NC)[i], ny1 = (s.y1 + cur * NC)[i];
          const int hx = (int)__builtin_ceilf((float)(nx1 - nx0) / 2);
          const int hy = (int)__builtin_ceilf((float)(ny1 - ny0) / 2);
          int rank = 0;
          for (int d = 0; d < 4; d++) {
            const int cc = s.ccnt[i * 4 + d];
            if (cc == 0) continue;
            const int p = (int)(pre & 0xFFFF) + rank++;
            const int ni = C - 1 - p;
            (s.x0 + nb * NC)[ni] = (int16_t)((d & 1) ? nx0 + hx : nx0);
            (s.x1 + nb * NC)[ni] = (int16_t)((d & 1) ? nx1 : nx0 + hx);
            (s.y0 + nb * NC)[ni] = (int16_t)((d & 2) ? ny0 + hy : ny0);
            (s.y1 + nb * NC)[ni] = (int16_t)((d & 2) ? ny1 : ny0 + hy);
            (s.cnt + nb * NC)[ni] = cc;
            (s.seq + nb * NC)[ni] = seqBase + p;
            s.cidx[i * 4 + d] = (int16_t)ni;
          }
        } else {
          const int ni = C + (int)((pre >> 16) & 0xFFFF);
          (s.x0 + nb * NC)[ni] = (s.x0 + cur * NC)[i];
          (s.x1 + nb * NC)[ni] = (s.x1 + cur * NC)[i];
          (s.y0 + nb * NC)[ni] = (s.y0 + cur * NC)[i];
          (s.y1 + nb * NC)[ni] = (s.y1 + cur * NC)[i];
          (s.cnt + nb * NC)[ni] = (s.cnt + cur * NC)[i];
          (s.seq + nb * NC)[ni] = (s.seq + cur * NC)[i];
          s.nidx[i] = (int16_t)ni;
        }
      }
      __syncthreads();
      oct_cands<NT>(T, oc, [&](int, uint32_t, uint32_t& nd) {
        const int n = (int)(nd & 0x3FFF);
        nd = (uint32_t)((s.cnt + cur * NC)[n] > 1 ? s.cidx[n * 4 + (nd >> 14)] : s.nidx[n]);
      });
      Snew = C + Sg;
      for (int i = tid; i < Snew * 4; i += NT) s.ccnt[i] = 0;
      seqBase += C;
      const bool finish = Snew >= N || Snew == S;
      S = Snew;
      cur = nb;
      if (finish) break;
      if (Snew + 3 * nexp > N) phase = 2;
    } else {
      for (int i = tid; i < S; i += NT) s.sa[i] = (s.cnt + cur * NC)[i] > 1 ? 1 : 0;
      __syncthreads();
      const int M = block_exclusive_scan<NT>(s.sa, S);
      const int P2 = next_pow2(max(M, 2));
      for (int i = tid; i < P2; i += NT) s.key[i] = 0;
      __syncthreads();
      for (int i = tid; i < S; i += NT)
        if ((s.cnt + cur * NC)[i] > 1)
          s.key[s.sa[i]] = ((uint64_t)(s.cnt + cur * NC)[i] << 43) | ((uint64_t)(s.seq + cur * NC)[i] << 13) | (uint64_t)i;
      __syncthreads();
      if (M <= kOctRankSortMax) {
        uint64_t* tmp = reinterpret_cast<uint64_t*>(s.cidx);
        for (int j = tid; j < M; j += NT) {
          const uint64_t x = s.key[j];
          int r = 0;
#pragma unroll 4
          for (int y = 0; y < M; y++) r += s.key[y] > x ? 1 : 0;
          tmp[r] = x;
        }
        __syncthreads();
        for (int j = tid; j < M; j += NT) s.key[j] = tmp[j];
        __syncthreads();
      } else {
        bitonic_sort_desc<NT>(s.key, P2);
      }
      if (tid == 0) s.ctrl[1] = M - 1;
      for (int j = tid; j < M; j += NT) {
        const int n = (int)(s.key[j] & 0x1FFF);
        int nc = 0;
        for (int d = 0; d < 4; d++) nc += s.ccnt[n * 4 + d] > 0;
        s.sb[j] = nc - 1;
      }
      __syncthreads();
      block_exclusive_scan<NT>(s.sb, M);
      for (int j = tid; j < M; j += NT) {
        const int n = (int)(s.key[j] & 0x1FFF);
        int nc = 0;
        for (int d = 0; d < 4; d++) nc += s.ccnt[n * 4 + d] > 0;
        if (S + s.sb[j] + (nc - 1) >= N) atomicMin(&s.ctrl[1], j);
      }
      __syncthreads();
      const int m = s.ctrl[1];
      for (int j = tid; j < M; j += NT) {
        int nc = 0;
        if (j <= m) {
          const int n = (int)(s.key[j] & 0x1FFF);
          for (int d = 0; d < 4; d++) nc += s.ccnt[n * 4 + d] > 0;
        }
        s.sb[j] = nc;
      }
      for (int i = tid; i < S; i += NT) s.nidx[i] = -1;
      __syncthreads();
      C = block_exclusive_scan<NT>(s.sb, M);
      for (int j = tid; j <= m; j += NT) {
        const int n = (int)(s.key[j] & 0x1FFF);
        s.nidx[n] = -2;
      }
      __syncthreads();
      for (int i = tid; i < S; i += NT) s.sa[i] = s.nidx[i] == -2 ? 0 : 1;
      __syncthreads();
      const int rest = block_exclusive_scan<NT>(s.sa, S);
      for (int j = tid; j <= m; j += NT) {
        const int i = (int)(s.key[j] & 0x1FFF);
        const int nx0 = (s.x0 + cur * NC)[i], ny0 = (s.y0 + cur * NC)[i], nx1 = (s.x1 + cur * NC)[i], ny1 = (s.y1 + cur * NC)[i];
        const int hx = (int)__builtin_ceilf((float)(nx1 - nx0) / 2);
        const int hy = (int)__builtin_ceilf((float)(ny1 - ny0) / 2);
        int rank = 0;
        for (int d = 0; d < 4; d++) {
          const int cc = s.ccnt[i * 4 + d];
          if (cc == 0) continue;
          const int p = s.sb[j] + rank++;
          const int ni = C - 1 - p;
          (s.x0 + nb * NC)[ni] = (int16_t)((d & 1) ? nx0 + hx : nx0);
          (s.x1 + nb * NC)[ni] = (int16_t)((d & 1) ? nx1 : nx0 + hx);
          (s.y0 + nb * NC)[ni] = (int16_t)((d & 2) ? ny0 + hy : ny0);
          (s.y1 + nb * NC)[ni] = (int16_t)((d & 2) ? ny1 : ny0 + hy);
          (s.cnt + nb * NC)[ni] = cc;
          (s.seq + nb * NC)[ni] = seqBase + p;
          s.cidx[i * 4 + d] = (int16_t)ni;
        }
      }
      for (int i = tid; i < S; i += NT) {
        if (s.nidx[i] == -2) continue;
        const int ni = C + s.sa[i];
        (s.x0 + nb * NC)[ni] = (s.x0 + cur * NC)[i];
        (s.x1 + nb * NC)[ni] = (s.x1 + cur * NC)[i];
        (s.y0 + nb * NC)[ni] = (s.y0 + cur * NC)[i];
        (s.y1 + nb * NC)[ni] = (s.y1 + cur * NC)[i];
        (s.cnt + nb * NC)[ni] = (s.cnt + cur * NC)[i];
        (s.seq + nb * NC)[ni] = (s.seq + cur * NC)[i];
        s.nidx[i] = (int16_t)ni;
      }
      __syncthreads();
      oct_cands<NT>(T, oc, [&](int, uint32_t, uint32_t& nd) {
        const int n = (int)(nd & 0x3FFF);
        const int ni = s.nidx[n];
        nd = (uint32_t)(ni == -2 ? s.cidx[n * 4 + (nd >> 14)] : ni);
      });
      Snew = C + rest;
      for (int i = tid; i < Snew * 4; i += NT) s.ccnt[i] = 0;
      seqBase += C;
      const bool finish = Snew >= N || Snew == S;
      S = Snew;
      cur = nb;
      if (finish) break;
    }
  }
  __syncthreads();
  OCT_TS(otf);
  for (int i = tid; i < S; i += NT) s.key[i] = 0;
  __syncthreads();
  oct_cands<NT>(T, oc, [&](int k, uint32_t v, uint32_t& nd) {
    const uint32_t x = (v & 0xFFF) + minBX, y = ((v >> 12) & 0xFFF) + minBY;
    const uint64_t key = ((uint64_t)(v >> 24) << 56) | ((uint64_t)(0xFFFFFFu - (uint32_t)k) << 24) |
                         (uint64_t)((y << 12) | x);
    atomicMax((unsigned long long*)&s.key[nd & 0x3FFF], (unsigned long long)key);
  });
  __syncthreads();
  const int nout = min(S, L.oct_cap);
  for (int i = tid; i < nout; i += NT) {
    const uint64_t key = s.key[i];
    oct_out[i] = ((uint32_t)(key >> 56) << 24) | (uint32_t)(key & 0xFFFFFF);
  }
  if (tid == 0) *oct_cnt = nout;
#ifdef ORBX_OCT_PROBE
  if (tid == 0 && oct_probe_buf) {
    const unsigned long long ot3 = __builtin_amdgcn_s_memtime();
    unsigned int* o = oct_probe_buf + ((size_t)img * G->nlevels + l) * kOctProbeWords;
    o[0] = (unsigned int)(ot1 - ot0);
    o[1] = (unsigned int)(ot2 - ot1);
    o[2] = (unsigned int)ot_p1;
    o[3] = (unsigned int)n_p1;
    o[4] = (unsigned int)ot_p2;
    o[5] = (unsigned int)n_p2;
    o[6] = (unsigned int)(ot3 - ot0);
    o[7] = (unsigned int)T;
    o[8] = (unsigned int)(ot3 - otf);
    o[9] = 2;
  }
#endif
  return 2;
}

template <int NT, class F>
__device__ __forceinline__ void oct_walk(const LevelGeom& L, const CellInfo* __restrict__ cells,
                                         const uint32_t* __restrict__ cand, const int* cpre, int T, F f) {
  const int tid = threadIdx.x, ncl = L.cell_end - L.cell_begin;
  if (ncl >= NT / 2) {
    for (int c = tid; c < ncl; c += NT) {
      const int k0 = cpre[c], n = cpre[c + 1] - k0;
      const CellInfo& ci = cells[L.cell_begin + c];
      const int kin = ci.kin, off = ci.cand_off, ovf = ci.ovf_off - kin;
      int i = 0;
      for (; i + 4 <= n; i += 4) {
        const uint32_t v0 = cand[(i < kin ? off : ovf) + i], v1 = cand[(i + 1 < kin ? off : ovf) + i + 1],
                       v2 = cand[(i + 2 < kin ? off : ovf) + i + 2], v3 = cand[(i + 3 < kin ? off : ovf) + i + 3];
        f(k0 + i, v0);
        f(k0 + i + 1, v1);
        f(k0 + i + 2, v2);
        f(k0 + i + 3, v3);
      }
      for (; i < n; i++) f(k0 + i, cand[(i < kin ? off : ovf) + i]);
    }
  } else {
    for (int k = tid; k < T; k += NT) {
      int lo = 0, hi = ncl - 1;
      while (lo < hi) {
        const int mid = (lo + hi + 1) >> 1;
        if (cpre[mid] <= k) lo = mid; else hi = mid - 1;
      }
      f(k, cand[cell_slot(cells[L.cell_begin + lo], k - cpre[lo])]);
    }
  }
}

template <int NT>
__device__ int oct_pyramid(const Geometry* __restrict__ G, const CellInfo* __restrict__ cells, const BatchPtrs& B,
                           const OctGroup& grp, int D, unsigned char* smem_raw, int img, int l) {
  const int tid = threadIdx.x;
  const LevelGeom& L = G->lv[l];
  const int NC = grp.node_cap;
  const int nIni = L.nIni;
  const OctPyrLayout lay = oct_pyr_layout(NC, grp.cell_cap, grp.pcap, grp.span, nIni, D);
  uint64_t* key = (uint64_t*)(smem_raw + lay.key);
  uint64_t* tmp = (uint64_t*)(smem_raw + lay.tmp);
  uint32_t* cell = (uint32_t*)(smem_raw + lay.cell);
  int* cnt = (int*)(smem_raw + lay.cnt);
  int* seq = (int*)(smem_raw + lay.seq);
  int* sa = (int*)(smem_raw + lay.sa);
  int* sb = (int*)(smem_raw + lay.sb);
  int* cpre = (int*)(smem_raw + lay.cpre);
  int* ctrl = (int*)(smem_raw + lay.ctrl);
  int16_t* nidx = (int16_t*)(smem_raw + lay.nidx);
  uint32_t* kp = (uint32_t*)(smem_raw + lay.kp);
  uint16_t* xtab = (uint16_t*)(smem_raw + lay.tab);
  uint32_t* pyrw = (uint32_t*)(smem_raw + lay.pyr);
  uint16_t* pyr = (uint16_t*)(smem_raw + lay.pyr);
  uint32_t* oct_out = B.oct + (size_t)img * G->oct_total + L.oct_off;
  int* oct_cnt = B.oct_count + (size_t)img * G->nlevels + l;

  OCT_TS(ot0);
#ifdef ORBX_OCT_PROBE
  unsigned long long ot_p1 = 0, ot_p2 = 0;
  int n_p1 = 0, n_p2 = 0;
#endif
  const int ncl = L.cell_end - L.cell_begin;
  for (int c = tid; c < ncl; c += NT) cpre[c] = B.cell_count[(size_t)img * G->ncells + L.cell_begin + c];
  __syncthreads();
  const int T = block_exclusive_scan<NT>(cpre, ncl);
  if (tid == 0) cpre[ncl] = T;
  if (T == 0) {
    if (tid == 0) *oct_cnt = 0;
    return 0;
  }
  if (T > 0xFFFF) return 2;
  const float hX = L.hX;
  const int minBX = L.minBX, minBY = L.minBY, boxH = max(L.maxBY - minBY, 1);
  const int npw = (oct_pyr_counters(nIni, D) + 1) / 2;
  for (int i = tid; i < npw; i += NT) pyrw[i] = 0;
  if (tid == 0) ctrl[0] = 0;
  const int boxW = max(L.maxBX - minBX, 1);
  uint16_t* ytab = xtab + boxW;
  for (int i = tid; i < boxW + boxH; i += NT) {
    int lo, hi, g = 0;
    const bool isx = i < boxW;
    const float f = (float)(isx ? i : i - boxW);
    if (isx) {
      g = (int)(f / hX);
      g = min(max(g, 0), nIni - 1);
      lo = (int)(hX * (float)g);
      hi = (int)(hX * (float)(g + 1));
    } else {
      lo = 0;
      hi = boxH;
    }
    for (int d = 0; d < D; d++) {
      const int h = (int)__builtin_ceilf((float)(hi - lo) / 2);
      const int q = f < (float)(lo + h) ? 0 : 1;
      if (q) lo += h; else hi = lo + h;
      g = 2 * g + q;
    }
    xtab[i] = (uint16_t)g;
  }
  __syncthreads();
  const uint32_t* cand = B.cand + (size_t)img * G->cand_total;
  const int offD = oct_pyr_off(nIni, D);
  auto leaf = [&](uint32_t v, int& gx, int& gy) {
    const int xr = (int)(v & 0xFFF) - minBX, yr = (int)((v >> 12) & 0xFFF) - minBY;
    gx = xtab[min(max(xr, 0), boxW - 1)];
    gy = ytab[min(max(yr, 0), boxH - 1)];
  };
  const int kcap = grp.pcap;
  oct_walk<NT>(L, cells, cand, cpre, T, [&](int k, uint32_t v) {
    int gx, gy;
    leaf(v, gx, gy);
    const int idx = offD + gy * (nIni << D) + gx;
    atomicAdd(&pyrw[idx >> 1], 1u << ((idx & 1) * 16));
    if (k < kcap) kp[k] = v;
  });
  __syncthreads();
  for (int d = D - 1; d >= 0; d--) {
    const int W = nIni << d, n = W << d, o = oct_pyr_off(nIni, d), oc = oct_pyr_off(nIni, d + 1);
    for (int c = tid; c < n; c += NT) {
      const int gy = c / W, gx = c - gy * W;
      const int ci = oc + 2 * gy * 2 * W + 2 * gx;
      const uint32_t w0 = pyrw[ci >> 1], w1 = pyrw[(ci + 2 * W) >> 1];
      pyr[o + c] = (uint16_t)((w0 & 0xFFFF) + (w0 >> 16) + (w1 & 0xFFFF) + (w1 >> 16));
    }
    __syncthreads();
  }
  OCT_TS(ot1);
  auto slot = [&](uint32_t c) {
    const int d = (int)(c >> 28);
    return oct_pyr_off(nIni, d) + (int)((c >> 20) & 0xFF) * (nIni << d) + (int)(c & 0xFFFFF);
  };
  auto kids = [&](uint32_t c, int* cc) {
    const int d = (int)(c >> 28) + 1, W = nIni << d;
    const int ci = oct_pyr_off(nIni, d) + 2 * (int)((c >> 20) & 0xFF) * W + 2 * (int)(c & 0xFFFFF);
    const uint32_t w0 = pyrw[ci >> 1], w1 = pyrw[(ci + W) >> 1];
    cc[0] = (int)(w0 & 0xFFFF);
    cc[1] = (int)(w0 >> 16);
    cc[2] = (int)(w1 & 0xFFFF);
    cc[3] = (int)(w1 >> 16);
  };
  auto child = [&](uint32_t c, int q) {
    return (((c >> 28) + 1) << 28) | ((2 * ((c >> 20) & 0xFF) + (uint32_t)(q >> 1)) << 20) |
           (2 * (c & 0xFFFFF) + (uint32_t)(q & 1));
  };
  constexpr uint16_t kSplit = 0xFFFF;
  for (int i = tid; i < nIni; i += NT) sa[i] = pyr[i] > 0 ? 1 : 0;
  __syncthreads();
  int S = block_exclusive_scan<NT>(sa, nIni);
  for (int i = tid; i < nIni; i += NT) {
    if (pyr[i] > 0) {
      const int ni = sa[i];
      cell[ni] = (uint32_t)i;
      cnt[ni] = pyr[i];
      seq[ni] = i;
    }
  }
  OCT_TS(ot2);
  int cur = 0;
  int seqBase = nIni;
  int phase = 1;
  const int N = L.nfeat;
  for (int round = 0; round < 256; round++) {
    __syncthreads();
#ifdef ORBX_OCT_PROBE
    const unsigned long long rt0 = __builtin_amdgcn_s_memtime();
    const int rphase = phase;
    struct RoundStamp {
      unsigned long long t0;
      int ph;
      unsigned long long *p1, *p2;
      int *n1, *n2;
      __device__ ~RoundStamp() {
        const unsigned long long d = __builtin_amdgcn_s_memtime() - t0;
        if (ph == 1) { *p1 += d; ++*n1; } else { *p2 += d; ++*n2; }
      }
    } rstamp{rt0, rphase, &ot_p1, &ot_p2, &n_p1, &n_p2};
#endif
    const int nb = cur ^ 1;
    const uint32_t* ccell = cell + cur * NC;
    const int *ccnt = cnt + cur * NC, *cseq = seq + cur * NC;
    uint32_t* ncell = cell + nb * NC;
    int *ncnt = cnt + nb * NC, *nseq = seq + nb * NC;
    int C, Snew;
    if (phase == 1) {
      for (int i = tid; i < S; i += NT) {
        uint64_t v = 1ull << 16;
        if (ccnt[i] > 1) {
          v = 0;
          if ((int)(ccell[i] >> 28) >= D) {
            ctrl[0] = 1;
          } else {
            int cc[4];
            kids(ccell[i], cc);
            for (int q = 0; q < 4; q++) v += (cc[q] > 0 ? 1ull : 0ull) + (cc[q] > 1 ? (1ull << 32) : 0ull);
          }
        }
        key[i] = v;
      }
      __syncthreads();
      if (ctrl[0]) return 2;
      const uint64_t tot = block_scan_excl<NT, uint64_t>(key, S);
      C = (int)(tot & 0xFFFF);
      const int Sg = (int)((tot >> 16) & 0xFFFF);
      const int nexp = (int)(tot >> 32);
      for (int i = tid; i < S; i += NT) {
        const uint64_t pre = key[i];
        if (ccnt[i] > 1) {
          const uint32_t c = ccell[i];
          int cc[4];
          kids(c, cc);
          int rank = 0;
          for (int q = 0; q < 4; q++) {
            if (cc[q] == 0) continue;
            const int p = (int)(pre & 0xFFFF) + rank++;
            const int ni = C - 1 - p;
            ncell[ni] = child(c, q);
            ncnt[ni] = cc[q];
            nseq[ni] = seqBase + p;
          }
          pyr[slot(c)] = kSplit;
        } else {
          const int ni = C + (int)((pre >> 16) & 0xFFFF);
          ncell[ni] = ccell[i];
          ncnt[ni] = ccnt[i];
          nseq[ni] = cseq[i];
        }
      }
      Snew = C + Sg;
      seqBase += C;
      const bool finish = Snew >= N || Snew == S;
      S = Snew;
      cur = nb;
      if (finish) break;
      if (Snew + 3 * nexp > N) phase = 2;
    } else {
      auto nchild = [&](int n) {
        if ((int)(ccell[n] >> 28) >= D) return 1;
        int cc[4];
        kids(ccell[n], cc);
        return (cc[0] > 0) + (cc[1] > 0) + (cc[2] > 0) + (cc[3] > 0);
      };
      for (int i = tid; i < S; i += NT) sa[i] = ccnt[i] > 1 ? 1 : 0;
      __syncthreads();
      const int M = block_exclusive_scan<NT>(sa, S);
      const int P2 = next_pow2(max(M, 2));
      for (int i = tid; i < P2; i += NT) key[i] = 0;
      __syncthreads();
      for (int i = tid; i < S; i += NT)
        if (ccnt[i] > 1) key[sa[i]] = ((uint64_t)ccnt[i] << 43) | ((uint64_t)cseq[i] << 13) | (uint64_t)i;
      __syncthreads();
      if (M <= kOctRankSortMax) {
        for (int j = tid; j < M; j += NT) {
          const uint64_t x = key[j];
          int r = 0;
#pragma unroll 4
          for (int y = 0; y < M; y++) r += key[y] > x ? 1 : 0;
          tmp[r] = x;
        }
        __syncthreads();
        for (int j = tid; j < M; j += NT) key[j] = tmp[j];
        __syncthreads();
      } else {
        bitonic_sort_desc<NT>(key, P2);
      }
      if (tid == 0) ctrl[1] = M - 1;
      for (int j = tid; j < M; j += NT) sb[j] = nchild((int)(key[j] & 0x1FFF)) - 1;
      __syncthreads();
      block_exclusive_scan<NT>(sb, M);
      for (int j = tid; j < M; j += NT) {
        const int nc = nchild((int)(key[j] & 0x1FFF));
        if (S + sb[j] + (nc - 1) >= N) atomicMin(&ctrl[1], j);
      }
      __syncthreads();
      const int m = ctrl[1];
      for (int j = tid; j < M; j += NT) {
        int nc = 0;
        if (j <= m) {
          const int n = (int)(key[j] & 0x1FFF);
          if ((int)(ccell[n] >> 28) >= D) ctrl[0] = 1;
          nc = nchild(n);
        }
        sb[j] = nc;
      }
      for (int i = tid; i < S; i += NT) nidx[i] = -1;
      __syncthreads();
      if (ctrl[0]) return 2;
      C = block_exclusive_scan<NT>(sb, M);
      for (int j = tid; j <= m; j += NT) nidx[(int)(key[j] & 0x1FFF)] = -2;
      __syncthreads();
      for (int i = tid; i < S; i += NT) sa[i] = nidx[i] == -2 ? 0 : 1;
      __syncthreads();
      const int rest = block_exclusive_scan<NT>(sa, S);
      for (int j = tid; j <= m; j += NT) {
        const int i = (int)(key[j] & 0x1FFF);
        const uint32_t c = ccell[i];
        int cc[4];
        kids(c, cc);
        int rank = 0;
        for (int q = 0; q < 4; q++) {
          if (cc[q] == 0) continue;
          const int p = sb[j] + rank++;
          const int ni = C - 1 - p;
          ncell[ni] = child(c, q);
          ncnt[ni] = cc[q];
          nseq[ni] = seqBase + p;
        }
        pyr[slot(c)] = kSplit;
      }
      for (int i = tid; i < S; i += NT) {
        if (nidx[i] == -2) continue;
        const int ni = C + sa[i];
        ncell[ni] = ccell[i];
        ncnt[ni] = ccnt[i];
        nseq[ni] = cseq[i];
      }
      Snew = C + rest;
      seqBase += C;
      const bool finish = Snew >= N || Snew == S;
      S = Snew;
      cur = nb;
      if (finish) break;
    }
  }
  __syncthreads();
  OCT_TS(otf);
  for (int i = tid; i < S; i += NT) {
    key[i] = 0;
    pyr[slot((cell + cur * NC)[i])] = (uint16_t)i;
  }
  __syncthreads();
  auto hand_over = [&](int k, uint32_t v) {
    int gx, gy;
    leaf(v, gx, gy);
    uint32_t nd = kSplit;
#pragma unroll
    for (int d = kOctMaxDepth; d >= 0; d--) {
      if (d > D) continue;
      const uint32_t c = pyr[oct_pyr_off(nIni, d) + (gy >> (D - d)) * (nIni << d) + (gx >> (D - d))];
      nd = c != kSplit ? c : nd;
    }
    const uint64_t kv = ((uint64_t)(v >> 24) << 56) | ((uint64_t)(0xFFFFFFu - (uint32_t)k) << 24) | (uint64_t)(v & 0xFFFFFF);
    if (nd < (uint32_t)S) atomicMax((unsigned long long*)&key[nd], (unsigned long long)kv);
  };
  if (T <= kcap) {
    for (int k = tid; k < T; k += NT) hand_over(k, kp[k]);
  } else {
    oct_walk<NT>(L, cells, cand, cpre, T, hand_over);
  }
  __syncthreads();
  const int nout = min(S, L.oct_cap);
  for (int i = tid; i < nout; i += NT) {
    const uint64_t kv = key[i];
    oct_out[i] = ((uint32_t)(kv >> 56) << 24) | (uint32_t)(kv & 0xFFFFFF);
  }
  if (tid == 0) *oct_cnt = nout;
#ifdef ORBX_OCT_PROBE
  if (tid == 0 && oct_probe_buf) {
    const unsigned long long ot3 = __builtin_amdgcn_s_memtime();
    unsigned int* o = oct_probe_buf + ((size_t)img * G->nlevels + l) * kOctProbeWords;
    o[0] = (unsigned int)(ot1 - ot0);
    o[1] = (unsigned int)(ot2 - ot1);
    o[2] = (unsigned int)ot_p1;
    o[3] = (unsigned int)n_p1;
    o[4] = (unsigned int)ot_p2;
    o[5] = (unsigned int)n_p2;
    o[6] = (unsigned int)(ot3 - ot0);
    o[7] = (unsigned int)T;
    o[8] = (unsigned int)(ot3 - otf);
    o[9] = 1;
  }
#endif
  return 1;
}

template <int NT>
__global__ __launch_bounds__(NT) __attribute__((amdgpu_waves_per_eu(6))) void k_octree(const Geometry* __restrict__ G, const CellInfo* __restrict__ cells,
                                               BatchPtrs B, OctGroup grp, int* __restrict__ path) {
  extern __shared__ __align__(16) unsigned char smem_raw[];
  const int img = blockIdx.x, l = grp.l0 + blockIdx.y;
  OCT_TS(kt0);
  int p = 2;
  if (grp.depth > 0) p = oct_pyramid<NT>(G, cells, B, grp, grp.depth, smem_raw, img, l);
  if (p == 2) {
    __syncthreads();
#ifdef ORBX_OCT_PROBE
    const unsigned long long kt1 = __builtin_amdgcn_s_memtime();
#endif
    p = oct_generic<NT>(G, cells, B, grp, smem_raw, img, l);
#ifdef ORBX_OCT_PROBE
    if (threadIdx.x == 0 && oct_probe_buf)
      oct_probe_buf[((size_t)img * G->nlevels + l) * kOctProbeWords + 10] = grp.depth > 0 ? (unsigned int)(kt1 - kt0) : 0;
#endif
  }
  if (path && threadIdx.x == 0) path[(size_t)img * G->nlevels + l] = p;
}

__device__ __forceinline__ int wave_sum_dpp(int v) {
  v += __builtin_amdgcn_update_dpp(0, v, 0x111, 0xF, 0xF, true);
  v += __builtin_amdgcn_update_dpp(0, v, 0x112, 0xF, 0xF, true);
  v += __builtin_amdgcn_update_dpp(0, v, 0x114, 0xF, 0xF, true);
  v += __builtin_amdgcn_update_dpp(0, v, 0x118, 0xF, 0xF, true);
  return __builtin_amdgcn_readlane(v, 15) + __builtin_amdgcn_readlane(v, 31) + __builtin_amdgcn_readlane(v, 47) +
         __builtin_amdgcn_readlane(v, 63);
}


constexpr int kPatchR = 18;
constexpr int kPatchRows = 2 * kPatchR + 1;
constexpr int kPS = 80;
constexpr int kDescLds = kPatchRows * kPS + 256;
struct PatchHW {
  int v[kPatchRows];
};
constexpr PatchHW kPatchHW = {{6,  8,  10, 11, 12, 13, 14, 15, 16, 16, 17, 17, 18, 18, 18, 18, 18, 18, 18,
                               18, 18, 18, 18, 18, 18, 17, 17, 16, 16, 15, 14, 13, 12, 11, 10, 8,  6}};
__constant__ PatchHW c_patch_hw = kPatchHW;
struct PatchSlots {
  uint8_t e[128];
};
constexpr int patch_row_chunks(int r) {
  int m = 0;
  for (int a = 0; a < 16; a++) {
    const int n = ((kPatchR + a + kPatchHW.v[r]) >> 4) - ((kPatchR + a - kPatchHW.v[r]) >> 4) + 1;
    m = n > m ? n : m;
  }
  return m;
}
constexpr PatchSlots make_patch_slots() {
  PatchSlots t{};
  for (int s = 0; s < 128; s++) t.e[s] = 0xFF;
  int n = 0, nrest = 0;
  uint8_t rest[12] = {};
  for (int ch = 0; ch < 4; ch++) {
    int rows[kPatchRows] = {}, nr = 0;
    for (int r = 0; r < kPatchRows; r++)
      if (patch_row_chunks(r) > ch) rows[nr++] = r;
    for (int q = 0; q + 4 <= nr; q += 4)
      for (int i = 0; i < 4; i++) t.e[n++] = (uint8_t)(rows[q + i] << 2 | ch);
    for (int q = nr & ~3; q < nr; q++) rest[nrest++] = (uint8_t)(rows[q] << 2 | ch);
  }
  for (int i = 0; i < nrest; i++) t.e[n++] = rest[i];
  return t;
}
constexpr PatchSlots kPatchSlots = make_patch_slots();
static_assert(kPatchSlots.e[123] != 0xFF && kPatchSlots.e[124] == 0xFF, "124 patch slots: two loads per lane");
__constant__ PatchSlots c_patch_slot = kPatchSlots;
const uint8_t* patch_slot_table() { return kPatchSlots.e; }

#ifndef ORBX_DESC_K
#define ORBX_DESC_K 8
#endif
constexpr int kDescK = ORBX_DESC_K;
static_assert(kDescK * 8 <= 64, "one descriptor dword per lane");

template <class F, int... I>
__device__ __forceinline__ void static_for_impl(F&& f, std::integer_sequence<int, I...>) {
  (f(std::integral_constant<int, I>{}), ...);
}
template <int N, class F>
__device__ __forceinline__ void static_for(F&& f) {
  static_for_impl(f, std::make_integer_sequence<int, N>{});
}
__device__ __forceinline__ const uint8_t* lane_ptr(const uint8_t* p, int j) {
  const uint64_t a = (uint64_t)p;
  const uint32_t lo = __builtin_amdgcn_readlane((uint32_t)a, j), hi = __builtin_amdgcn_readlane((uint32_t)(a >> 32), j);
  return (const uint8_t*)(((uint64_t)hi << 32) | lo);
}
__device__ __forceinline__ float lane_f(float v, int j) {
  return __builtin_bit_cast(float, __builtin_amdgcn_readlane(__builtin_bit_cast(int, v), j));
}

__global__ __launch_bounds__(BS) void k_describe(const Geometry* __restrict__ G, BatchPtrs B,
                                                 orbx_keypoint* __restrict__ kps, uint8_t* __restrict__ desc,
                                                 int32_t* __restrict__ counts, int kp_cap, XcdRemap R) {
  __shared__ __align__(16) uint8_t s_desc[BS / 64][kDescLds];
  const int2 bi = xcd_block2(R);
  const int img = bi.y;
  const int lane = threadIdx.x & 63, wv = threadIdx.x >> 6;
  const int i0 = __builtin_amdgcn_readfirstlane((bi.x * (BS / 64) + wv) * kDescK);
  const int nl = G->nlevels;
  const int* oc = B.oct_count + (size_t)img * nl;
  int cnt[kMaxLevelsPlan];
#pragma unroll
  for (int ll = 0; ll < kMaxLevelsPlan; ll++) cnt[ll] = ll < nl ? oc[ll] : 0;
  int total = 0;
#pragma unroll
  for (int ll = 0; ll < kMaxLevelsPlan; ll++) total += cnt[ll];
  if (bi.x == 0 && threadIdx.x == 0) counts[img] = total;
  float4 pat[4];
#pragma unroll
  for (int k = 0; k < 4; k++) pat[k] = reinterpret_cast<const float4*>(c_pattern_f)[lane + 64 * k];
  if (i0 >= total) return;
  const int nk = min(kDescK, total - i0);
  const int i = i0 + min(lane, nk - 1);
  int l = 0, first = 0, acc = 0;
#pragma unroll
  for (int ll = 0; ll < kMaxLevelsPlan; ll++) {
    if (i >= acc) {
      l = ll;
      first = acc;
// ... 276 lines not shown
```

orb_slam2_commit_amd/csrc/orbx_extractor.h:

```cpp
#pragma once
#include <hip/hip_runtime.h>

#include <algorithm>
#include <cstring>
#include <map>
#include <memory>
#include <utility>

#include "orbx_mem.h"
#include "orbx_plan.h"
#include "orbx_prof.h"
#include "orbx_scratch.h"
#include "orbx_stereo.h"

namespace orbx {

struct DevPlan : Plan {
  LaunchPlan LP{};
  DevBuf<Geometry> dG;
  DevBuf<CellInfo> dcells;
  DevBuf<int> dtiles;
  DevBuf<ResizeX> dxt;
  DevBuf<ResizeY> dyt;
  DevBuf<int2> drzb;
};

struct BlockCursor {
  size_t at = 256;
  template <class T>
  size_t take(size_t count) {
    const size_t o = at;
    at += scratch_align(count * sizeof(T));
    return o;
  }
  size_t end() const { return at; }
};

inline void pack_rows(uint8_t* dst, const void* src, size_t stride, size_t row_bytes, int rows) {
  for (int y = 0; y < rows; y++) std::memcpy(dst + (size_t)y * row_bytes, (const uint8_t*)src + (size_t)y * stride, row_bytes);
}

inline void copy_out(void* dst, const void* src, size_t bytes) {
  if (dst) std::memcpy(dst, src, bytes);
}

struct StereoSide {
  const orbx_keypoint* kps;
  const uint8_t* desc;
  const int32_t* counts;
  long long k_stride, n_stride;
  int step, off;
};
struct StereoSides {
  StereoSide L, R;
  static StereoSides handles(const orbx_keypoint* kL, const uint8_t* dL, const int32_t* nL, const orbx_keypoint* kR,
                             const uint8_t* dR, const int32_t* nR) {
    return {{kL, dL, nL, 0, 0, 0, 0}, {kR, dR, nR, 0, 0, 0, 0}};
  }
  static StereoSides interleaved(const orbx_keypoint* kps, const uint8_t* desc, const int32_t* counts, long long kc) {
    return {{kps, desc, counts, 2 * kc, 2, 2, 0}, {kps + kc, desc + kc * 32, counts + 1, 2 * kc, 2, 2, 1}};
  }
};

}

struct orbx_extractor {
  orbx_extractor_params params{};
  int device = 0;
  hipStream_t stream = nullptr;
  orbx::Tables tables;
  std::map<std::pair<int, int>, std::unique_ptr<orbx::DevPlan>> plans;
  orbx::DevBuf<uint8_t> pyr, blur;
  orbx::DevBuf<uint32_t> cand, kpos, oct;
  orbx::DevBuf<int> cell_count, knode, oct_count;
  orbx::DevBuf<uint8_t> in, out;
  size_t out_kps = 0, out_desc = 0, out_bytes = 0;
  orbx::PinnedBuf hstage;
  orbx::DevBuf<uint64_t> rkeys;
  orbx::DevBuf<int2> rxi;
  orbx::DevBuf<uint4> rdesc;
  orbx::DevBuf<uint32_t> rtab;
  orbx::DevBuf<uint4> lrange;
  orbx::DevBuf<int> oct_start, sad;
  orbx::DevBuf<float> sres;
  orbx::DevBuf<int32_t> nmatch;
  orbx::DevBuf<uint8_t> rgbd_in;
  orbx::DevBuf<int32_t> rgbd_oob;
  orbx::StageTimer timer;
  orbx::DevPlan* last_plan = nullptr;
  const uint8_t* last_in = nullptr;
  size_t last_pitch = 0;
  int last_n = 0;
  bool last_host = false;
  int last_fp_n = 0;
  uint64_t last_fp = 0;
  bool pyr_readback = false;
  bool hpyr_valid = false;
  orbx::PinnedBuf hpyr;
  size_t hpyr_l0 = 0;
};

namespace orbx {

inline orbx_status hip_status(hipError_t e) { return e == hipSuccess ? ORBX_OK : ORBX_ERR_HIP; }
inline hipStream_t pick_stream(orbx_extractor* h, void* s) {
  return s == ORBX_STREAM_NULL ? (hipStream_t)0 : s ? (hipStream_t)s : h->stream;
}
orbx_status get_plan(orbx_extractor* h, int W, int H, DevPlan** out);
orbx_status ensure_batch(orbx_extractor* h, const Plan& P, int n);
BatchPtrs batch_ptrs(orbx_extractor* h, const uint8_t* in, size_t pitch);
orbx_status run_extract(orbx_extractor* h, DevPlan* P, int n, const uint8_t* d_in, size_t pitch, orbx_keypoint* d_kps,
                        uint8_t* d_desc, int32_t* d_counts, int kp_cap, hipStream_t st);
orbx_status run_stereo(orbx_extractor* hl, orbx_extractor* hr, int n_frames, const StereoSides& S, int maxL, float bf,
                       float baseline, float* uR, float* depth, long long out_stride, int32_t* nmatches,
                       hipStream_t st);

}
```

orb_slam2_commit_amd/csrc/orbx_stereo.h:

```cpp
#pragma once
#include "orbx_internal.h"

namespace orbx {

constexpr int kMaxStereoKps = 4096;

struct StereoArgs {
  const orbx_keypoint* kpL;
  const uint8_t* dL;
  const int32_t* nL;
  long long kL_stride;
  long long n_stride_L;
  const orbx_keypoint* kpR;
  const uint8_t* dR;
  const int32_t* nR;
  long long kR_stride;
  long long n_stride_R;
  BatchPtrs BL, BR;
  int l_step, l_off, r_step, r_off;
  int nlevels;
  int maxL;
  float inv_scale[kMaxLevelsPlan];
  float bf, minZ, minD, maxD;
  float* uR;
  float* depth;
  int* sad;
  long long out_stride;
  uint64_t* rkeys;
  int* oct_start;
  int2* rxi;
  uint4* rdesc;
  uint32_t* rtab;
  uint4* lrange;
  int rows;
  int32_t* nmatches;
};

struct StageTimer;
hipError_t launch_stereo(const StereoArgs& A, const Geometry* Gd, int n_frames, int maxL, hipStream_t st,
                         StageTimer* T);
hipError_t launch_hamming(const uint8_t* a, const uint8_t* b, int n, int32_t* out, hipStream_t st);

}
```

orb_slam2_commit_amd/csrc/stereo.hip:

```cpp
#include <hip/hip_runtime.h>

#include "orbx_device.h"
#include "orbx_internal.h"
#include "orbx_stereo.h"
#include "orbx_prof.h"

namespace orbx {

constexpr int SBS = 256;
typedef unsigned short u16x2 __attribute__((ext_vector_type(2)));

__device__ __forceinline__ uint32_t fbits(float f) { return __float_as_uint(f); }

constexpr int PBS = 1024;
__global__ __launch_bounds__(PBS) void k_stereo_prep(StereoArgs A, const Geometry* __restrict__ G) {
  __shared__ uint64_t keys[kMaxStereoKps];
  __shared__ int ost[kMaxLevelsPlan + 1];
  const int f = blockIdx.x, tid = threadIdx.x;
  const int nR = min(A.nR[(size_t)f * A.n_stride_R], kMaxStereoKps);
  const orbx_keypoint* kR = A.kpR + (size_t)f * A.kR_stride;
  int P2 = 2;
  while (P2 < nR) P2 <<= 1;
  for (int i = tid; i < P2; i += PBS) {
    uint64_t k = ~0ull;
    if (i < nR) {
      const orbx_keypoint kp = kR[i];
      k = ((uint64_t)(uint32_t)kp.octave << 44) | ((uint64_t)fbits(kp.y) << 12) | (uint64_t)i;
    }
    keys[i] = k;
  }
  __syncthreads();
  for (int size = 2; size <= P2; size <<= 1) {
    for (int stride = size >> 1; stride > 0; stride >>= 1) {
      for (int i = tid; i < P2 / 2; i += PBS) {
        const int lo = 2 * i - (i & (stride - 1));
        const int hi = lo + stride;
        const bool asc = (lo & size) == 0;
        const uint64_t a = keys[lo], b = keys[hi];
        if (asc ? (a > b) : (a < b)) {
          keys[lo] = b;
          keys[hi] = a;
        }
      }
      __syncthreads();
    }
  }
  uint64_t* out = A.rkeys + (size_t)f * kMaxStereoKps;
  int2* rxi = A.rxi + (size_t)f * kMaxStereoKps;
  for (int i = tid; i < nR; i += PBS) {
    const uint64_t k = keys[i];
    out[i] = k;
    const int idx = (int)(k & 0xFFF);
    rxi[i] = make_int2(__float_as_int(kR[idx].x), idx);
  }
  {
    const uint4* dR = (const uint4*)(A.dR + (size_t)f * A.kR_stride * 32);
    uint4* rd = A.rdesc + (size_t)f * kMaxStereoKps * 2;
    for (int e = tid; e < 2 * nR; e += PBS) rd[e] = dR[2 * (int)(keys[e >> 1] & 0xFFF) + (e & 1)];
  }
  int* os = A.oct_start + (size_t)f * (kMaxLevelsPlan + 1);
  for (int o = tid; o <= A.nlevels; o += PBS) {
    int lo = 0, hi = nR;
    while (lo < hi) {
      const int mid = (lo + hi) >> 1;
      if ((int)(keys[mid] >> 44) < o) lo = mid + 1; else hi = mid;
    }
    os[o] = lo;
    ost[o] = lo;
  }
  __syncthreads();
  uint32_t* tab = A.rtab + (size_t)f * A.nlevels * A.rows;
  for (int e = tid; e < A.nlevels * A.rows; e += PBS) {
    const int o = e / A.rows, Y = e - o * A.rows;
    const float r = 2.0f * G->lv[o].scale;
    const int lo = ost[o], hi = ost[o + 1];
    int a = lo, b = hi;
    while (a < b) {
      const int m = (a + b) >> 1;
      if ((int)__builtin_ceilf(__uint_as_float((uint32_t)(keys[m] >> 12)) + r) >= Y) b = m; else a = m + 1;
    }
    int c = a, d = hi;
    while (c < d) {
      const int m = (c + d) >> 1;
      if ((int)__builtin_floorf(__uint_as_float((uint32_t)(keys[m] >> 12)) - r) > Y) d = m; else c = m + 1;
    }
    tab[e] = (uint32_t)a | ((uint32_t)c << 16);
  }
  __syncthreads();
  const int nL = min(A.nL[(size_t)f * A.n_stride_L], A.maxL);
  const orbx_keypoint* kL = A.kpL + (size_t)f * A.kL_stride;
  uint4* lr = A.lrange + (size_t)f * A.maxL;
  for (int i = tid; i < nL; i += PBS) {
    const orbx_keypoint kp = kL[i];
    const int Y = (int)kp.y;
    uint32_t t[3];
#pragma unroll
    for (int q = 0; q < 3; q++) {
      const int o = kp.octave - 1 + q;
      t[q] = (o >= 0 && o < A.nlevels && Y >= 0 && Y < A.rows) ? tab[(size_t)o * A.rows + Y] : 0u;
    }
    lr[i] = make_uint4(t[0], t[1], t[2], 0u);
  }
}

constexpr int kKpsPerBlock = SBS / 16;
constexpr int kSadDwL = 4, kSadDwR = 6, kSadDw = kSadDwL + kSadDwR;

__device__ __forceinline__ uint32_t row_min_u32(uint32_t v) {
  v = min(v, (uint32_t)__builtin_amdgcn_update_dpp(0, (int)v, 0x128, 0xF, 0xF, false));
  v = min(v, (uint32_t)__builtin_amdgcn_update_dpp(0, (int)v, 0x124, 0xF, 0xF, false));
  v = min(v, (uint32_t)__builtin_amdgcn_update_dpp(0, (int)v, 0x122, 0xF, 0xF, false));
  v = min(v, (uint32_t)__builtin_amdgcn_update_dpp(0, (int)v, 0x121, 0xF, 0xF, false));
  return v;
}

#ifdef ORBX_STEREO_ROWS_PROBE
constexpr int kProbeFrames = 512, kProbeKps = 2048;
__device__ uint2 g_rows_probe[kProbeFrames * kProbeKps];
constexpr int kProbeWords = 1 << 20;
__device__ uint32_t g_probe_bits[4][kProbeWords];
__device__ unsigned long long g_probe_count[3];
#endif

__global__ __launch_bounds__(SBS, 8) void k_stereo_match(StereoArgs A, const Geometry* __restrict__ G, XcdRemap R) {
  constexpr int NQ = SBS / 16;
  __shared__ uint32_t s_raw[NQ][11 * kSadDw];
  __shared__ uint32_t s_sw[NQ][66 + 121];
  const int2 bi = xcd_block2(R);
  const int f = bi.y, tid = threadIdx.x, lane = tid & 63, ql = lane & 15, qb = tid >> 4;
  const int nL = min(A.nL[(size_t)f * A.n_stride_L], A.maxL);
  const int iL = bi.x * NQ + qb;
  if (iL >= nL) return;
  const int2* rxi = A.rxi + (size_t)f * kMaxStereoKps;
  const uint4* rdR = A.rdesc + (size_t)f * kMaxStereoKps * 2;
  const orbx_keypoint* kL = A.kpL + (size_t)f * A.kL_stride;
  const int limg = f * A.l_step + A.l_off, rimg = f * A.r_step + A.r_off;
  const orbx_keypoint kp = kL[iL];
  const uint4 lrg = A.lrange[(size_t)f * A.maxL + iL];
  uint64_t ld[4];
  {
    const uint64_t* p = (const uint64_t*)(A.dL + ((size_t)f * A.kL_stride + iL) * 32);
    ld[0] = p[0]; ld[1] = p[1]; ld[2] = p[2]; ld[3] = p[3];
  }
  const int levelL = kp.octave;
  const float uL = kp.x;
  const float minU = uL - A.maxD, maxU = uL - A.minD;
  float* outU = A.uR + (size_t)f * A.out_stride + iL;
  float* outD = A.depth + (size_t)f * A.out_stride + iL;
  int* outS = A.sad + (size_t)f * A.out_stride + iL;
  if (ql == 0) {
    *outU = -1.0f;
    *outD = -1.0f;
    *outS = -1;
  }
#ifdef ORBX_STEREO_ROWS_PROBE
  if (ql == 0 && f < kProbeFrames && iL < kProbeKps) g_rows_probe[f * kProbeKps + iL] = make_uint2(0u, 0u);
#endif
  if (maxU < 0) return;
  const uint32_t t3[3] = {lrg.x, lrg.y, lrg.z};
  int rb[3], re[3];
#pragma unroll
  for (int q = 0; q < 3; q++) {
    rb[q] = (int)(t3[q] & 0xFFFF);
    re[q] = (int)(t3[q] >> 16);
  }
  const int n0 = re[0] - rb[0], n1 = re[1] - rb[1], n2 = re[2] - rb[2];
  const int K = n0 + n1 + n2;
  uint32_t best = 0xFFFFFFFFu;
  float bestX = 0.f;
  for (int j = ql; j < K; j += 16) {
    const int pos = j < n0 ? rb[0] + j : (j < n0 + n1 ? rb[1] + (j - n0) : rb[2] + (j - n0 - n1));
    const int2 xi = rxi[pos];
    const uint4 r0 = rdR[2 * pos], r1 = rdR[2 * pos + 1];
    const float uR = __int_as_float(xi.x);
    if (!(uR >= minU && uR <= maxU)) continue;
    const uint64_t rd[4] = {(uint64_t)r0.x | ((uint64_t)r0.y << 32), (uint64_t)r0.z | ((uint64_t)r0.w << 32),
                            (uint64_t)r1.x | ((uint64_t)r1.y << 32), (uint64_t)r1.z | ((uint64_t)r1.w << 32)};
    const int dist = hamming256(ld, rd);
    const uint32_t key = ((uint32_t)dist << 12) | (uint32_t)xi.y;
    if (key < best) {
      best = key;
      bestX = uR;
    }
  }
  const uint32_t wbest = row_min_u32(best);
  const int bestDist = wbest == 0xFFFFFFFFu ? 100 : (int)(wbest >> 12);
  if (bestDist >= 75) return;
  const LevelGeom& Lv = G->lv[levelL];
  const uint64_t om = __ballot(best == wbest) >> (lane & 48);
  const int owner = (lane & 48) + __builtin_ctzll(om & 0xFFFF);
  const float uR0 = __shfl(bestX, owner, 64);
  const float sf = A.inv_scale[levelL];
  const float scaleduL = __builtin_roundf(kp.x * sf);
  const float scaledvL = __builtin_roundf(kp.y * sf);
  const float scaleduR0 = __builtin_roundf(uR0 * sf);
  const int w = 5, L = 5;
  const float iniu = scaleduR0 + L - w;
  const float endu = scaleduR0 + L + w + 1;
  if (iniu < 0 || endu >= Lv.w) return;
  if (scaleduR0 - 2 * w < 0 || scaledvL - w < 0 || scaledvL + w >= Lv.h || scaleduL - w < 0 ||
      scaleduL + w >= Lv.w)
    return;
  const uint8_t* imL = level_ptr(*G, A.BL, limg, levelL);
  const uint8_t* imR = level_ptr(*G, A.BR, rimg, levelL);
  const int lw = Lv.w;
  const int cy = (int)scaledvL, cxL = (int)scaleduL, cxR0 = (int)scaleduR0;
  uint32_t* sp = s_raw[qb];
  const uint8_t* rowL0 = imL + (size_t)(cy - w) * lw + (cxL - w);
  const uint8_t* rowR0 = imR + (size_t)(cy - w) * lw + (cxR0 - 2 * w);
#ifdef ORBX_STEREO_ROWS_PROBE
  if (ql == 0 && f < kProbeFrames && iL < kProbeKps)
    g_rows_probe[f * kProbeKps + iL] = make_uint2((uint32_t)(rowL0 - imL), (uint32_t)(rowR0 - imR) + 1u);
#endif
  {
    constexpr int IT = (11 * kSadDw + 15) / 16;
    uint32_t sv[IT];
#pragma unroll
    for (int k = 0; k < IT; k++) {
      const int q = ql + 16 * k, r = q / kSadDw, j = q - r * kSadDw;
      const bool left = j < kSadDwL;
      const uintptr_t a = (uintptr_t)((left ? rowL0 : rowR0) + (size_t)r * lw);
      const int jj = left ? j : j - kSadDwL, need = left ? 2 * w + 1 : 4 * w + 1;
      sv[k] = 0;
      if (q < 11 * kSadDw && 4 * jj < (int)(a & 3) + need) sv[k] = *((const uint32_t*)(a & ~(uintptr_t)3) + jj);
    }
#pragma unroll
    for (int k = 0; k < IT; k++)
      if (ql + 16 * k < 11 * kSadDw) sp[ql + 16 * k] = sv[k];
  }
  __builtin_amdgcn_fence(__ATOMIC_RELEASE, "wavefront");
  __builtin_amdgcn_wave_barrier();
  __builtin_amdgcn_fence(__ATOMIC_ACQUIRE, "wavefront");
  const uint8_t* sb = reinterpret_cast<const uint8_t*>(sp);
  const uint32_t aL0 = (uint32_t)(uintptr_t)rowL0, aR0 = (uint32_t)(uintptr_t)rowR0;
  auto lpix = [&](int dy, int dx) -> int { return sb[4 * kSadDw * dy + ((aL0 + (uint32_t)(dy * lw)) & 3) + dx]; };
  auto rpix = [&](int dy, int dx) -> int {
    return sb[4 * (kSadDw * dy + kSadDwL) + ((aR0 + (uint32_t)(dy * lw)) & 3) + dx];
  };
  uint32_t* l16 = s_sw[qb];
  uint32_t* re16 = l16 + 66;
  const uint32_t Lc = (uint32_t)lpix(w, w);
  for (int q = ql; q < 66; q += 16) {
    const int r = q / 6, k = q - r * 6;
    l16[q] = (uint32_t)lpix(r, 2 * k) | (2 * k + 1 <= 2 * w ? (uint32_t)lpix(r, 2 * k + 1) << 16 : 0u);
  }
  for (int q = ql; q < 121; q += 16) {
    const int r = q / 11, k = q - r * 11;
    const uint32_t a = (uint32_t)rpix(r, 2 * k) + Lc;
    const uint32_t b = (2 * k + 1 <= 4 * w ? (uint32_t)rpix(r, 2 * k + 1) : 0u) + Lc;
    re16[q] = a | b << 16;
  }
  __builtin_amdgcn_fence(__ATOMIC_RELEASE, "wavefront");
  __builtin_amdgcn_wave_barrier();
  __builtin_amdgcn_fence(__ATOMIC_ACQUIRE, "wavefront");
  const int so = ql < 11 ? ql : 0;
  const uint32_t rc = (uint32_t)rpix(w, so + w);
  const u16x2 rc2 = {(uint16_t)rc, (uint16_t)rc};
  const uint32_t* rrow = re16 + (so >> 1);
  const uint32_t sh = (uint32_t)(so & 1) * 2;
  uint32_t acc = 0;
#pragma unroll
  for (int dy = 0; dy < 2 * w + 1; dy++) {
    uint32_t wv[7];
#pragma unroll
    for (int t = 0; t < 7; t++) wv[t] = rrow[dy * 11 + t];
#pragma unroll
    for (int p2 = 0; p2 < 6; p2++) {
      uint32_t lp = __builtin_bit_cast(uint32_t, __builtin_bit_cast(u16x2, l16[dy * 6 + p2]) + rc2);
      uint32_t rp = __builtin_amdgcn_alignbyte(wv[p2 + 1], wv[p2], sh);
      if (p2 == 5) {
        lp &= 0xFFFFu;
        rp &= 0xFFFFu;
      }
      acc = __builtin_amdgcn_sad_u16(lp, rp, acc);
    }
  }
  const int sad = (int)acc;
  const uint32_t skey = row_min_u32(ql < 11 ? ((uint32_t)sad << 4) | (uint32_t)ql : 0xFFFFFFFFu);
  const int bix = (int)(skey & 15);
  const int bestSad = (int)(skey >> 4);
  const int bestinc = bix - L;
  const int qbase = lane & 48;
  const float d1 = (float)__shfl(sad, qbase + max(bix - 1, 0), 64);
  const float d3 = (float)__shfl(sad, qbase + min(bix + 1, 15), 64);
  if (bestinc == -L || bestinc == L) return;
  const float d2 = (float)bestSad;
  const float deltaR = (d1 - d3) / (2.0f * (d1 + d3 - 2.0f * d2));
  if (deltaR < -1 || deltaR > 1) return;
  float bestuR = Lv.scale * ((float)scaleduR0 + (float)bestinc + deltaR);
  float disparity = uL - bestuR;
  if (disparity >= A.minD && disparity < A.maxD) {
    if (disparity <= 0) {
      disparity = 0.01f;
      bestuR = uL - 0.01f;
    }
    if (ql == 0) {
      *outD = A.bf / disparity;
      *outU = bestuR;
      *outS = bestSad;
    }
  }
}

__global__ __launch_bounds__(SBS) void k_stereo_finalize(StereoArgs A) {
  __shared__ int hist[256];
  __shared__ int sel[4];
  const int f = blockIdx.x, tid = threadIdx.x;
  const int nL = min(A.nL[(size_t)f * A.n_stride_L], A.maxL);
  const int* sad = A.sad + (size_t)f * A.out_stride;
  float* uR = A.uR + (size_t)f * A.out_stride;
  float* depth = A.depth + (size_t)f * A.out_stride;
  for (int i = tid; i < 256; i += SBS) hist[i] = 0;
  __syncthreads();
  for (int i = tid; i < nL; i += SBS) {
    const int s = sad[i];
    if (s >= 0) atomicAdd(&hist[(s >> 8) & 255], 1);
  }
  __syncthreads();
  if (tid == 0) {
    int n = 0;
    for (int b = 0; b < 256; b++) n += hist[b];
    sel[0] = n;
    const int k = n / 2;
    int acc = 0, b = 0;
    for (; b < 256; b++) {
      if (acc + hist[b] > k) break;
      acc += hist[b];
    }
    sel[1] = b;
    sel[2] = k - acc;
  }
  __syncthreads();
  const int n = sel[0];
  if (n == 0) {
    if (tid == 0) A.nmatches[f] = 0;
    return;
  }
  const int hb = sel[1], k2 = sel[2];
  __syncthreads();
  for (int i = tid; i < 256; i += SBS) hist[i] = 0;
  __syncthreads();
  for (int i = tid; i < nL; i += SBS) {
    const int s = sad[i];
    if (s >= 0 && ((s >> 8) & 255) == hb) atomicAdd(&hist[s & 255], 1);
  }
  __syncthreads();
  if (tid == 0) {
    int acc = 0, b = 0;
    for (; b < 256; b++) {
      if (acc + hist[b] > k2) break;
      acc += hist[b];
    }
    sel[3] = (hb << 8) | b;
  }
  __syncthreads();
  const float median = (float)sel[3];
  const float th = 1.5f * 1.4f * median;
  int kept = 0;
  for (int i = tid; i < nL; i += SBS) {
    const int s = sad[i];
    if (s < 0) continue;
    if ((float)s >= th) {
      uR[i] = -1.0f;
      depth[i] = -1.0f;
    } else {
      kept++;
    }
  }
  kept = wave_sum(kept);
  __shared__ int ksum;
  if (tid == 0) ksum = 0;
  __syncthreads();
  if ((tid & 63) == 0) atomicAdd(&ksum, kept);
  __syncthreads();
  if (tid == 0) A.nmatches[f] = ksum;
}

__global__ __launch_bounds__(SBS) void k_hamming(const uint8_t* __restrict__ a, const uint8_t* __restrict__ b, int n,
                                                 int32_t* __restrict__ out) {
  const int i = blockIdx.x * SBS + threadIdx.x;
  if (i >= n) return;
  const uint64_t* pa = (const uint64_t*)(a + (size_t)i * 32);
  const uint64_t* pb = (const uint64_t*)(b + (size_t)i * 32);
  uint64_t x[4] = {pa[0], pa[1], pa[2], pa[3]};
  uint64_t y[4] = {pb[0], pb[1], pb[2], pb[3]};
  out[i] = hamming256(x, y);
}

#ifdef ORBX_STEREO_ROWS_PROBE
template <typename Fn>
__device__ inline void probe_rows(const StereoArgs& A, const Geometry* G, int f, int iL, int ql, Fn fn) {
  const uint2 rec = g_rows_probe[f * kProbeKps + iL];
  if (rec.y == 0) return;
  const orbx_keypoint kp = (A.kpL + (size_t)f * A.kL_stride)[iL];
  const int limg = f * A.l_step + A.l_off, rimg = f * A.r_step + A.r_off;
  const uint8_t* rowL0 = level_ptr(*G, A.BL, limg, kp.octave) + rec.x;
  const uint8_t* rowR0 = level_ptr(*G, A.BR, rimg, kp.octave) + (rec.y - 1u);
  const int lw = G->lv[kp.octave].w, w = 5;
  constexpr int IT = (11 * kSadDw + 15) / 16;
#pragma unroll
  for (int k = 0; k < IT; k++) {
    const int q = ql + 16 * k, r = q / kSadDw, j = q - r * kSadDw;
    const bool left = j < kSadDwL;
    const uintptr_t a = (uintptr_t)((left ? rowL0 : rowR0) + (size_t)r * lw);
    const int jj = left ? j : j - kSadDwL, need = left ? 2 * w + 1 : 4 * w + 1;
    if (q < 11 * kSadDw && 4 * jj < (int)(a & 3) + need)
      fn(left ? 0 : 1, kp.octave == 0, (a & ~(uintptr_t)3) + 4 * (uintptr_t)jj);
  }
}

__global__ __launch_bounds__(SBS) void k_stereo_rows_only(StereoArgs A, const Geometry* __restrict__ G, uint32_t* sink, XcdRemap R) {
  constexpr int NQ = SBS / 16;
  const int2 bi = xcd_block2(R);
  const int f = bi.y, tid = threadIdx.x, ql = tid & 15, qb = tid >> 4;
  const int nL = min(A.nL[(size_t)f * A.n_stride_L], A.maxL);
  const int iL = bi.x * NQ + qb;
  if (iL >= nL || f >= kProbeFrames || iL >= kProbeKps) return;
  uint32_t x = 0;
  probe_rows(A, G, f, iL, ql, [&](int, bool, uintptr_t a) { x ^= *(const uint32_t*)a; });
  if (x == 0x9E3779B9u) sink[0] = x;
}

__device__ inline void probe_mark(const StereoArgs& A, int side, bool l0, uintptr_t a) {
  const BatchPtrs& B = side ? A.BR : A.BL;
  const int m = 2 * side + (l0 ? 0 : 1);
  const uintptr_t off = a - (l0 ? (uintptr_t)B.in : (uintptr_t)B.pyr);
  const unsigned long long sec = off >> 6;
  if (sec < 32ull * kProbeWords) atomicOr(&g_probe_bits[m][sec >> 5], 1u << (sec & 31));
}

__global__ __launch_bounds__(SBS) void k_stereo_rows_mark(StereoArgs A, const Geometry* __restrict__ G) {
  constexpr int NQ = SBS / 16;
  const int f = blockIdx.y, tid = threadIdx.x, ql = tid & 15, qb = tid >> 4;
  const int nL = min(A.nL[(size_t)f * A.n_stride_L], A.maxL);
  const int iL = blockIdx.x * NQ + qb;
  if (iL >= nL || f >= kProbeFrames || iL >= kProbeKps) return;
  if (ql == 0 && g_rows_probe[f * kProbeKps + iL].y) atomicAdd(&g_probe_count[2], 1ull);
  probe_rows(A, G, f, iL, ql, [&](int side, bool l0, uintptr_t a) { probe_mark(A, side, l0, a); });
}

__global__ __launch_bounds__(256) void k_stereo_rows_count() {
  unsigned long long s = 0, l = 0;
  for (int i = blockIdx.x * 256 + threadIdx.x; i < 4 * kProbeWords; i += gridDim.x * 256) {
    uint32_t* wp = &g_probe_bits[i / kProbeWords][i % kProbeWords];
    const uint32_t v = *wp;
    if (v) {
      s += __popc(v);
      l += __popc((v | (v >> 1)) & 0x55555555u);
      *wp = 0;
    }
  }
  for (int o = 32; o > 0; o >>= 1) {
    s += __shfl_down(s, o, 64);
    l += __shfl_down(l, o, 64);
  }
  if ((threadIdx.x & 63) == 0 && (s || l)) {
    atomicAdd(&g_probe_count[0], s);
    atomicAdd(&g_probe_count[1], l);
  }
}
#endif

hipError_t launch_stereo(const StereoArgs& A, const Geometry* Gd, int n_frames, int maxL, hipStream_t st,
                         StageTimer* T) {
  T->begin(st);
  hipLaunchKernelGGL(k_stereo_prep, dim3(n_frames), dim3(PBS), 0, st, A, Gd);
  T->end(ST_STEREO_PREP, st);
  const int nb = (maxL + kKpsPerBlock - 1) / kKpsPerBlock;
  XcdRemap R;
  if (!make_xcd_remap(max(nb, 1), n_frames, 1, &R)) return hipErrorInvalidValue;
  T->begin(st);
  hipLaunchKernelGGL(k_stereo_match, dim3(max(nb, 1), n_frames), dim3(SBS), 0, st, A, Gd, R);
  T->end(ST_STEREO_MATCH, st);
  T->begin(st);
  hipLaunchKernelGGL(k_stereo_finalize, dim3(n_frames), dim3(SBS), 0, st, A);
  T->end(ST_STEREO_FINAL, st);
#ifdef ORBX_STEREO_ROWS_PROBE
  hipLaunchKernelGGL(k_stereo_rows_only, dim3(max(nb, 1), n_frames), dim3(SBS), 0, st, A, Gd, (uint32_t*)A.nmatches, R);
  hipLaunchKernelGGL(k_stereo_rows_mark, dim3(max(nb, 1), n_frames), dim3(SBS), 0, st, A, Gd);
  hipLaunchKernelGGL(k_stereo_rows_count, dim3(1024), dim3(256), 0, st);
#endif
  return hipGetLastError();
}

hipError_t launch_hamming(const uint8_t* a, const uint8_t* b, int n, int32_t* out, hipStream_t st) {
  if (n <= 0) return hipSuccess;
  hipLaunchKernelGGL(k_hamming, dim3((n + SBS - 1) / SBS), dim3(SBS), 0, st, a, b, n, out);
  return hipGetLastError();
}

}

#ifdef ORBX_STEREO_ROWS_PROBE
extern "C" int orbx_debug_stereo_floor(unsigned long long* out) {
  if (hipDeviceSynchronize() != hipSuccess) return -1;
  unsigned long long h[3] = {0, 0, 0};
  if (hipMemcpyFromSymbol(h, HIP_SYMBOL(orbx::g_probe_count), sizeof(h)) != hipSuccess) return -1;
  const unsigned long long z[3] = {0, 0, 0};
  if (hipMemcpyToSymbol(HIP_SYMBOL(orbx::g_probe_count), z, sizeof(z)) != hipSuccess) return -1;
  for (int i = 0; i < 3; i++) out[i] = h[i];
  return 0;
}
#endif
```

orb_slam2_commit_amd/orb.py:

```python
import contextlib
import ctypes as C
import threading

import numpy as np

from . import _lib
from ._lib import KEYPOINT_DTYPE, check, ptr

TH_HIGH = 100
TH_LOW = 50
HISTO_LENGTH = 30


class ORBextractor:

    def __init__(self, nfeatures, scaleFactor, nlevels, iniThFAST, minThFAST, device=0):
        L = _lib.lib()
        self.params = _lib.ExtractorParams(int(nfeatures), float(scaleFactor), int(nlevels), int(iniThFAST),
                                           int(minThFAST))
        h = C.c_void_p()
        check(L.orbx_extractor_create(C.byref(self.params), int(device), C.byref(h)), "orbx_extractor_create")
        self._h = h
        self.nfeatures = int(nfeatures)
        self.scaleFactor = float(scaleFactor)
        self.nlevels = int(nlevels)
        self.device = int(device)
        n = self.nlevels
        self._tables = [np.zeros(n, np.float32) for _ in range(4)]
        check(L.orbx_extractor_scale_tables(h, *[ptr(t) for t in self._tables]), "orbx_extractor_scale_tables")
        self._last_shape = None

    def close(self):
        if getattr(self, "_h", None):
            _lib.lib().orbx_extractor_destroy(self._h)
            self._h = None

    def __del__(self):
        try:
            self.close()
        except Exception:
            pass

    def GetLevels(self):
        return _lib.lib().orbx_extractor_get_levels(self._h)

    def GetScaleFactor(self):
        return self.scaleFactor

    def GetScaleFactors(self):
        return self._tables[0].copy()

    def GetInverseScaleFactors(self):
        return self._tables[1].copy()

    def GetScaleSigmaSquares(self):
        return self._tables[2].copy()

    def GetInverseScaleSigmaSquares(self):
        return self._tables[3].copy()

    def max_keypoints(self, width, height):
        n = _lib.lib().orbx_extractor_max_keypoints(self._h, int(width), int(height))
        if n < 0:
            check(n, "orbx_extractor_max_keypoints")
        return n

    def __call__(self, image, mask=None):
        if image is None or getattr(image, "size", 0) == 0:
            return np.zeros(0, KEYPOINT_DTYPE), None
        img = np.asarray(image)
        assert img.dtype == np.uint8 and img.ndim == 2, "image must be CV_8UC1"
        h, w = img.shape
        if img.strides[1] != 1:
            img = np.ascontiguousarray(img)
        cap = self.max_keypoints(w, h)
        kps = np.zeros(cap, KEYPOINT_DTYPE)
        desc = np.zeros((cap, 32), np.uint8)
        n = C.c_int(0)
        check(_lib.lib().orbx_extract(self._h, ptr(img), w, h, img.strides[0], ptr(kps), cap, ptr(desc), C.byref(n)),
              "orbx_extract")
        self._last_shape = (w, h)
        n = n.value
        if n == 0:
            return kps[:0].copy(), None
        return kps[:n].copy(), desc[:n].copy()

    @property
    def mvImagePyramid(self):
        return [self.pyramid_level(l) for l in range(self.nlevels)]

    def pyramid_level(self, level, image=0):
        L = _lib.lib()
        w, h = C.c_int(0), C.c_int(0)
        check(L.orbx_pyramid_level(self._h, image, level, None, 0, C.byref(w), C.byref(h)), "orbx_pyramid_level")
        out = np.zeros((h.value, w.value), np.uint8)
        check(L.orbx_pyramid_level(self._h, image, level, ptr(out), w.value, C.byref(w), C.byref(h)),
              "orbx_pyramid_level")
        return out

    def extract_batch_device(self, images, kps, desc, counts, stream=None):
        n, h, w = images.shape
        cap = kps.shape[1]
        check(_lib.lib().orbx_extract_batch_device(self._h, n, ptr(images), w, h, h * w, ptr(kps), ptr(desc),
                                                   ptr(counts), cap, _stream_ptr(stream, True)),
              "orbx_extract_batch_device")

    def stereo_frames_device(self, images, kps, desc, counts, bf, baseline, uright, depth, nmatches, stream=None):
        n2, h, w = images.shape
        cap = kps.shape[1]
        check(_lib.lib().orbx_stereo_frames_device(self._h, n2 // 2, ptr(images), w, h, h * w, ptr(kps), ptr(desc),
                                                   ptr(counts), cap, C.c_float(bf), C.c_float(baseline),
                                                   ptr(uright), ptr(depth), ptr(nmatches), _stream_ptr(stream, True)),
              "orbx_stereo_frames_device")


def _stream_ptr(stream, handle_api=False):
    if stream is None:
        return None
    s = stream.cuda_stream if hasattr(stream, "cuda_stream") else int(stream)
    if s == 0 and handle_api:
        return C.c_void_p(1)
    return C.c_void_p(s)


def compute_stereo_matches(extractor_left, extractor_right, kps_left, desc_left, kps_right, desc_right, bf,
                           baseline):
    nL, nR = len(kps_left), len(kps_right)
    uR = np.full(nL, -1.0, np.float32)
    depth = np.full(nL, -1.0, np.float32)
    if nL == 0:
        return uR, depth
    kL = np.ascontiguousarray(kps_left, KEYPOINT_DTYPE)
    kR = np.ascontiguousarray(kps_right, KEYPOINT_DTYPE)
    dL = np.ascontiguousarray(desc_left, np.uint8)
    dR = np.ascontiguousarray(desc_right if desc_right is not None else np.zeros((0, 32), np.uint8), np.uint8)
    check(_lib.lib().orbx_stereo_match(extractor_left._h, extractor_right._h, ptr(kL), ptr(dL), nL, ptr(kR),
                                       ptr(dR), nR, C.c_float(bf), C.c_float(baseline), ptr(uR), ptr(depth)),
          "orbx_stereo_match")
    return uR, depth


def debug_stereo_keypoints(extractor_left, extractor_right, kps_left, desc_left, kps_right, desc_right, bf,
                           baseline):
    nL, nR = len(kps_left), len(kps_right)
    uR = np.full(nL, -1.0, np.float32)
    depth = np.full(nL, -1.0, np.float32)
    sad = np.full(nL, -1, np.int32)
    nm = np.zeros(1, np.int32)
    kL = np.ascontiguousarray(kps_left, KEYPOINT_DTYPE)
    kR = np.ascontiguousarray(kps_right, KEYPOINT_DTYPE)
    dL = np.ascontiguousarray(desc_left if desc_left is not None else np.zeros((0, 32), np.uint8), np.uint8)
    dR = np.ascontiguousarray(desc_right if desc_right is not None else np.zeros((0, 32), np.uint8), np.uint8)
    assert dL.shape == (nL, 32) and dR.shape == (nR, 32)
    check(_lib.lib().orbx_debug_stereo_keypoints(extractor_left._h, extractor_right._h, ptr(kL), ptr(dL), nL,
                                                 ptr(kR), ptr(dR), nR, C.c_float(bf), C.c_float(baseline), ptr(uR),
                                                 ptr(depth), ptr(sad), ptr(nm)),
          "orbx_debug_stereo_keypoints")
    return uR, depth, sad, int(nm[0])


def debug_launch_plan(params, width, height, what, a0=0, a1=0, a2=0):
    L = _lib.lib()
    n = L.orbx_debug_launch_plan(C.byref(params), int(width), int(height), int(what), a0, a1, a2, None, 0)
    if n < 0:
        check(n, "orbx_debug_launch_plan")
    out = np.zeros(n, np.int64)
    L.orbx_debug_launch_plan(C.byref(params), int(width), int(height), int(what), a0, a1, a2, ptr(out), n)
    return out


def debug_octree_candidates(extractor, cell_counts, candidates):
    counts = np.ascontiguousarray(cell_counts, np.int32)
    cand = np.ascontiguousarray(candidates, np.uint32)
    w, h = extractor._last_shape
    cells = debug_launch_plan(extractor.params, w, h, 11).reshape(-1, 8)
    levels = debug_launch_plan(extractor.params, w, h, 12).reshape(-1, 8)
    n_img = len(counts)
    assert counts.shape == (n_img, len(cells)) and cand.shape == (n_img, int(cells[:, 6].sum()))
    oct_count = np.zeros((n_img, extractor.nlevels), np.int32)
    oct_out = np.zeros((n_img, int(levels[:, 7].sum())), np.uint32)
    check(_lib.lib().orbx_debug_octree_candidates(extractor._h, n_img, ptr(counts), ptr(cand), ptr(oct_count),
                                                  ptr(oct_out)), "orbx_debug_octree_candidates")
    return oct_count, oct_out


def debug_octree_paths(extractor, cell_counts, candidates, depth_cap=-1):
    counts = np.ascontiguousarray(cell_counts, np.int32)
    cand = np.ascontiguousarray(candidates, np.uint32)
    w, h = extractor._last_shape
    cells = debug_launch_plan(extractor.params, w, h, 11).reshape(-1, 8)
    levels = debug_launch_plan(extractor.params, w, h, 12).reshape(-1, 8)
    n_img = len(counts)
    assert counts.shape == (n_img, len(cells)) and cand.shape == (n_img, int(cells[:, 6].sum()))
    oct_count = np.zeros((n_img, extractor.nlevels), np.int32)
    oct_out = np.zeros((n_img, int(levels[:, 7].sum())), np.uint32)
    paths = np.zeros((n_img, extractor.nlevels), np.int32)
    check(_lib.lib().orbx_debug_octree_paths(extractor._h, n_img, ptr(counts), ptr(cand), int(depth_cap),
                                             ptr(oct_count), ptr(oct_out), ptr(paths)), "orbx_debug_octree_paths")
    return oct_count, oct_out, paths


def frame_stereo(extractor, image_left, image_right, bf, baseline):
    L = np.asarray(image_left)
    R = np.asarray(image_right)
    assert L.dtype == np.uint8 and L.ndim == 2 and R.dtype == np.uint8 and R.shape == L.shape, "two CV_8UC1 images"
    if L.strides[1] != 1:
        L = np.ascontiguousarray(L)
    if R.strides[1] != 1:
        R = np.ascontiguousarray(R)
    h, w = L.shape
    cap = extractor.max_keypoints(w, h)
    kL, kR = np.zeros(cap, KEYPOINT_DTYPE), np.zeros(cap, KEYPOINT_DTYPE)
    dL, dR = np.zeros((cap, 32), np.uint8), np.zeros((cap, 32), np.uint8)
    uR, depth = np.full(cap, -1.0, np.float32), np.full(cap, -1.0, np.float32)
    nL, nR = C.c_int(0), C.c_int(0)
    check(_lib.lib().orbx_frame_stereo(extractor._h, ptr(L), L.strides[0], ptr(R), R.strides[0], w, h, C.c_float(bf),
                                       C.c_float(baseline), ptr(kL), ptr(dL), cap, C.byref(nL), ptr(kR), ptr(dR), cap,
                                       C.byref(nR), ptr(uR), ptr(depth)),
          "orbx_frame_stereo")
    extractor._last_shape = (w, h)
    nL, nR = nL.value, nR.value
    return (kL[:nL].copy(), dL[:nL].copy() if nL else None, kR[:nR].copy(), dR[:nR].copy() if nR else None,
            uR[:nL].copy(), depth[:nL].copy())


def cvt_gray(image, rgb, device=0):
    a = np.asarray(image)
    assert a.dtype == np.uint8 and a.ndim in (3, 4), "image must be CV_8UC3 / CV_8UC4 (or a batch of them)"
    b = a if a.ndim == 4 else a[None]
    n, h, w, c = b.shape
    if b.size and (b.strides[3] != 1 or b.strides[2] != c or b.strides[1] < w * c or
                   (n > 1 and b.strides[0] < (h - 1) * b.strides[1] + w * c)):
        b = np.ascontiguousarray(b)
    out = np.zeros((n, h, w), np.uint8)
    check(_lib.lib().orbx_cvt_gray(ptr(b), b.strides[1], b.strides[0], n, w, h, c, int(bool(rgb)), ptr(out), w,
                                   w * h, int(device)), "orbx_cvt_gray")
    return out if a.ndim == 4 else out[0]


def _depth_type(depth):
    if depth.dtype == np.uint16:
        return _lib.ORBX_DEPTH_U16
    if depth.dtype == np.float32:
        return _lib.ORBX_DEPTH_F32
    raise TypeError("depth image must be CV_16U or CV_32F, not %s" % depth.dtype)


def frame_rgbd(extractor, image, depth, depth_factor, K, dist_coef, bf, rgb=True):
    img = np.asarray(image)
    dep = np.asarray(depth)
    assert img.dtype == np.uint8 and img.ndim in (2, 3), "image must be CV_8UC1 / C3 / C4"
    ch = 1 if img.ndim == 2 else img.shape[2]
    if img.size and (img.strides[1] != ch or (img.ndim == 3 and img.strides[2] != 1)):
        img = np.ascontiguousarray(img)
    assert dep.ndim == 2
    if dep.size and dep.strides[1] != dep.itemsize:
        dep = np.ascontiguousarray(dep)
    h, w = img.shape[:2]
    cap = max(extractor.max_keypoints(w, h), 1) if w > 0 and h > 0 else 1
    kps, kun = np.zeros(cap, KEYPOINT_DTYPE), np.zeros(cap, KEYPOINT_DTYPE)
    desc = np.zeros((cap, 32), np.uint8)
    uR, d = np.full(cap, -1.0, np.float32), np.full(cap, -1.0, np.float32)
    n = C.c_int(0)
    cam = camera(K, dist_coef)
    check(_lib.lib().orbx_frame_rgbd(extractor._h, ptr(img) if img.size else None, img.strides[0], w, h, ch,
                                     int(bool(rgb)), ptr(dep), dep.strides[0], dep.shape[1], dep.shape[0],
                                     _depth_type(dep), C.c_float(depth_factor), C.byref(cam), C.c_float(bf),
                                     ptr(kps), ptr(desc), cap, C.byref(n), ptr(kun), ptr(uR), ptr(d)),
          "orbx_frame_rgbd")
    extractor._last_shape = (w, h)
    n = n.value
    return kps[:n].copy(), desc[:n].copy() if n else None, kun[:n].copy(), uR[:n].copy(), d[:n].copy()


def rgbd_frames_device(extractor, images, depth, depth_factor, K, dist_coef, bf, kps, desc, counts, kps_un, uright,
                       depth_out, nmatches, rgb=True, stream=None):
    n, h, w = images.shape[:3]
    ch = 1 if images.dim() == 3 else images.shape[3]
    assert images.stride(2) == ch and (ch == 1 or images.stride(3) == 1) and depth.stride(2) == 1
    es = depth.element_size()
    dtype = _lib.ORBX_DEPTH_U16 if es == 2 else _lib.ORBX_DEPTH_F32
    assert es == 2 or depth.is_floating_point(), "depth must be 16-bit integer or float32"
    cam = camera(K, dist_coef)
    check(_lib.lib().orbx_rgbd_frames_device(extractor._h, n, ptr(images), w, h, ch, int(bool(rgb)), images.stride(1),
                                             images.stride(0), ptr(depth), dtype, depth.stride(1) * es,
                                             depth.stride(0) * es, C.c_float(depth_factor), C.byref(cam),
                                             C.c_float(bf), ptr(kps), ptr(desc), ptr(counts), kps.shape[1],
                                             ptr(kps_un), ptr(uright), ptr(depth_out), ptr(nmatches),
                                             _stream_ptr(stream, True)),
          "orbx_rgbd_frames_device")


def compute_distinctive_descriptors(desc, obs_off, device=0):
    d = np.ascontiguousarray(desc, np.uint8).reshape(-1, 32)
    off = np.ascontiguousarray(obs_off, np.int32)
    n = len(off) - 1
    best = np.zeros(max(n, 1), np.int32)
    out = np.zeros((max(n, 1), 32), np.uint8)
    check(_lib.lib().orbx_distinctive_descriptors(ptr(d), ptr(off), n, ptr(best), ptr(out), int(device)),
          "orbx_distinctive_descriptors")
    return best[:n], out[:n]


def camera(K, dist_coef):
    d = np.asarray(dist_coef, np.float32).reshape(-1)
    cam = _lib.Camera()
    cam.K[:] = _f32(K).reshape(9).tolist()
    dd = np.zeros(5, np.float32)
    dd[:len(d)] = d
    cam.dist[:] = dd.tolist()
    cam.n_dist = len(d)
# ... 1410 lines not shown
```

Measured before the change: 120,300 frames/s.

## Bin-sort stereo right keypoints, parallel median select, cache octree cell table

```diff
diff --git a/include/orbx_debug.h b/include/orbx_debug.h
--- a/include/orbx_debug.h
+++ b/include/orbx_debug.h
@@ -41,6 +41,10 @@
                                         int nR, float bf, float baseline, float* uRight, float* depth, int32_t* sad,
                                         int32_t* nmatches);
 int orbx_debug_stereo_keypoints_check(const orbx_keypoint* kps, int n, int nlevels, int width, int height);
+orbx_status orbx_debug_stereo_prep(orbx_extractor* h, const orbx_keypoint* kpsR, int nR, int32_t* order,
+                                   int32_t* oct_start, uint32_t* rtab);
+orbx_status orbx_debug_stereo_median(const int32_t* sad, int n, float* uRight, float* depth, int32_t* nmatches,
+                                     int device);
 
 orbx_status orbx_debug_octree_candidates(orbx_extractor* h, int n_img, const int32_t* cell_counts,
                                          const uint32_t* candidates, int32_t* oct_count, uint32_t* oct_out);
diff --git a/orb_slam2_commit_amd/_lib.py b/orb_slam2_commit_amd/_lib.py
--- a/orb_slam2_commit_amd/_lib.py
+++ b/orb_slam2_commit_amd/_lib.py
@@ -388,6 +388,8 @@
                                 C.c_size_t], C.c_longlong),
     "orbx_debug_stereo_keypoints": ([P, P, P, P, C.c_int, P, P, C.c_int, C.c_float, C.c_float, P, P, P, P], C.c_int),
     "orbx_debug_stereo_keypoints_check": ([P, C.c_int, C.c_int, C.c_int, C.c_int], C.c_int),
+    "orbx_debug_stereo_prep": ([P, P, C.c_int, P, P, P], C.c_int),
+    "orbx_debug_stereo_median": ([P, C.c_int, P, P, P, C.c_int], C.c_int),
     "orbx_debug_octree_candidates": ([P, C.c_int, P, P, P, P], C.c_int),
     "orbx_debug_octree_paths": ([P, C.c_int, P, P, C.c_int, P, P, P], C.c_int),    "orbx_debug_octree_candidates_check": ([C.POINTER(ExtractorParams), C.c_int, C.c_int, C.c_int, P, P], C.c_int),
     "orbx_debug_atan2_det": ([C.c_double, C.c_double], C.c_double),
@@ -424,7 +426,7 @@
 BA_CAPTURE_HEADER = ("fired", "phase", "it", "q", "ok", "trial", "nc", "np", "ne", "na", "npa", "nposes")
 
 _lib = None
-_NEWER_ENTRIES = {"orbx_debug_octree_paths"}
+_NEWER_ENTRIES = {"orbx_debug_octree_paths", "orbx_debug_stereo_prep", "orbx_debug_stereo_median"}
 
 
 def lib():
diff --git a/orb_slam2_commit_amd/csrc/capi.hip b/orb_slam2_commit_amd/csrc/capi.hip
--- a/orb_slam2_commit_amd/csrc/capi.hip
+++ b/orb_slam2_commit_amd/csrc/capi.hip
@@ -92,7 +92,6 @@
   const DevPlan* P = hl->last_plan;
   hipError_t e = hipSuccess;
   auto chk = [&](hipError_t x) { if (x != hipSuccess) e = x; };
-  chk(h->rkeys.ensure((size_t)n_frames * kMaxStereoKps));
   chk(h->oct_start.ensure((size_t)n_frames * (kMaxLevelsPlan + 1)));
   chk(h->rxi.ensure((size_t)n_frames * kMaxStereoKps));
   chk(h->rdesc.ensure((size_t)n_frames * kMaxStereoKps * 2));
@@ -129,7 +128,6 @@
   A.depth = depth;
   A.sad = h->sad.p;
   A.out_stride = out_stride;
-  A.rkeys = h->rkeys.p;
   A.oct_start = h->oct_start.p;
   A.rxi = h->rxi.p;
   A.rdesc = h->rdesc.p;
diff --git a/orb_slam2_commit_amd/csrc/debug.hip b/orb_slam2_commit_amd/csrc/debug.hip
--- a/orb_slam2_commit_amd/csrc/debug.hip
+++ b/orb_slam2_commit_amd/csrc/debug.hip
@@ -175,6 +175,91 @@
   return hip_status(e);
 }
 
+extern "C" orbx_status orbx_debug_stereo_prep(orbx_extractor* h, const orbx_keypoint* kpsR, int nR, int32_t* order,
+                                              int32_t* oct_start, uint32_t* rtab) {
+  if (!h || !order || !oct_start || !rtab || nR < 0 || (nR > 0 && !kpsR)) return ORBX_ERR_ARG;
+  if (nR > kMaxStereoKps) return ORBX_ERR_CAPACITY;
+  if (!h->last_plan) return ORBX_ERR_STATE;
+  const DevPlan& P = *h->last_plan;
+  const int nlevels = P.G.nlevels, rows = std::max(P.G.height, 1);
+  if (hipSetDevice(h->device) != hipSuccess) return ORBX_ERR_HIP;
+  BlockCursor cur;
+  const size_t o_kR = cur.take<orbx_keypoint>(nR), o_dR = cur.take<uint8_t>((size_t)nR * 32),
+               o_os = cur.take<int>(kMaxLevelsPlan + 1), o_rxi = cur.take<int2>(kMaxStereoKps),
+               o_rd = cur.take<uint4>((size_t)kMaxStereoKps * 2), o_tab = cur.take<uint32_t>((size_t)nlevels * rows),
+               o_lr = cur.take<uint4>(1);
+  DevBuf<uint8_t> blk;
+  if (blk.ensure(cur.end()) != hipSuccess) return ORBX_ERR_HIP;
+  hipError_t e = hipSuccess;
+  auto chk = [&](hipError_t x) { if (x != hipSuccess) e = x; };
+  hipStream_t st = h->stream;
+  const int32_t counts[3] = {0, nR, 0};
+  chk(hipMemcpyAsync(blk.p, counts, sizeof(counts), hipMemcpyHostToDevice, st));
+  if (nR > 0) {
+    chk(hipMemcpyAsync(blk.p + o_kR, kpsR, (size_t)nR * sizeof(orbx_keypoint), hipMemcpyHostToDevice, st));
+    chk(hipMemsetAsync(blk.p + o_dR, 0, (size_t)nR * 32, st));
+  }
+  StereoArgs A;
+  std::memset(&A, 0, sizeof(A));
+  A.kpL = (const orbx_keypoint*)(blk.p + o_kR);
+  A.nL = (const int32_t*)blk.p;
+  A.kpR = (const orbx_keypoint*)(blk.p + o_kR);
+  A.dR = blk.p + o_dR;
+  A.nR = (const int32_t*)blk.p + 1;
+  A.nlevels = nlevels;
+  A.maxL = 1;
+  A.rows = rows;
+  A.oct_start = (int*)(blk.p + o_os);
+  A.rxi = (int2*)(blk.p + o_rxi);
+  A.rdesc = (uint4*)(blk.p + o_rd);
+  A.rtab = (uint32_t*)(blk.p + o_tab);
+  A.lrange = (uint4*)(blk.p + o_lr);
+  if (e == hipSuccess) chk(launch_stereo_prep(A, P.dG.p, 1, st));
+  std::vector<int2> rxi((size_t)nR);
+  if (e == hipSuccess) {
+    if (nR > 0) chk(hipMemcpyAsync(rxi.data(), blk.p + o_rxi, sizeof(int2) * nR, hipMemcpyDeviceToHost, st));
+    chk(hipMemcpyAsync(oct_start, blk.p + o_os, sizeof(int) * (nlevels + 1), hipMemcpyDeviceToHost, st));
+    chk(hipMemcpyAsync(rtab, blk.p + o_tab, sizeof(uint32_t) * nlevels * rows, hipMemcpyDeviceToHost, st));
+  }
+  chk(hipStreamSynchronize(st));
+  for (int i = 0; i < nR; i++) order[i] = rxi[i].y;
+  return hip_status(e);
+}
+
+extern "C" orbx_status orbx_debug_stereo_median(const int32_t* sad, int n, float* uRight, float* depth,
+                                                int32_t* nmatches, int device) {
+  if (n < 0 || !nmatches || (n > 0 && (!sad || !uRight || !depth))) return ORBX_ERR_ARG;
+  *nmatches = 0;
+  if (n == 0) return ORBX_OK;
+  if (hipSetDevice(device) != hipSuccess) return ORBX_ERR_HIP;
+  BlockCursor cur;
+  const size_t o_sad = cur.take<int32_t>(n), o_ur = cur.take<float>(n), o_dep = cur.take<float>(n);
+  DevBuf<uint8_t> blk;
+  if (blk.ensure(cur.end()) != hipSuccess) return ORBX_ERR_HIP;
+  hipError_t e = hipSuccess;
+  auto chk = [&](hipError_t x) { if (x != hipSuccess) e = x; };
+  const int32_t counts[2] = {n, 0};
+  chk(hipMemcpy(blk.p, counts, sizeof(counts), hipMemcpyHostToDevice));
+  chk(hipMemcpy(blk.p + o_sad, sad, sizeof(int32_t) * n, hipMemcpyHostToDevice));
+  chk(hipMemcpy(blk.p + o_ur, uRight, sizeof(float) * n, hipMemcpyHostToDevice));
+  chk(hipMemcpy(blk.p + o_dep, depth, sizeof(float) * n, hipMemcpyHostToDevice));
+  StereoArgs A;
+  std::memset(&A, 0, sizeof(A));
+  A.nL = (const int32_t*)blk.p;
+  A.maxL = n;
+  A.sad = (int*)(blk.p + o_sad);
+  A.uR = (float*)(blk.p + o_ur);
+  A.depth = (float*)(blk.p + o_dep);
+  A.out_stride = n;
+  A.nmatches = (int32_t*)blk.p + 1;
+  if (e == hipSuccess) chk(launch_stereo_finalize(A, 1, nullptr));
+  if (e == hipSuccess) chk(hipMemcpy(uRight, blk.p + o_ur, sizeof(float) * n, hipMemcpyDeviceToHost));
+  if (e == hipSuccess) chk(hipMemcpy(depth, blk.p + o_dep, sizeof(float) * n, hipMemcpyDeviceToHost));
+  if (e == hipSuccess) chk(hipMemcpy(nmatches, blk.p + 4, sizeof(int32_t), hipMemcpyDeviceToHost));
+  chk(hipDeviceSynchronize());
+  return hip_status(e);
+}
+
 constexpr int kOctInjectMaxImages = 64;
 static bool octree_candidates_ok(const Plan& P, int n_img, const int32_t* counts, const uint32_t* cand) {
   const Geometry& G = P.G;
diff --git a/orb_slam2_commit_amd/csrc/extract.hip b/orb_slam2_commit_amd/csrc/extract.hip
--- a/orb_slam2_commit_amd/csrc/extract.hip
+++ b/orb_slam2_commit_amd/csrc/extract.hip
@@ -949,6 +949,62 @@
 #define OCT_TS(v)
 #endif
 
+constexpr int kOctWalkChunk = 8;
+__host__ __device__ inline bool oct_cell_table_fits(int ncl, int NC) { return 3 * ncl * 4 <= 16 * NC; }
+
+template <int NT>
+__device__ __forceinline__ void oct_stage_cells(const CellInfo* __restrict__ lc, const int* __restrict__ count, int ncl,
+                                                int* cpre, int* tab) {
+  for (int c = threadIdx.x; c < ncl; c += NT) {
+    const int n = count ? count[c] : 0;
+    if (tab) {
+      const CellInfo& ci = lc[c];
+      const int kin = ci.kin, off = ci.cand_off, ovf = ci.ovf_off;
+      tab[c] = off;
+      tab[ncl + c] = ovf - kin;
+      tab[2 * ncl + c] = kin;
+    }
+    if (count) cpre[c] = n;
+  }
+}
+
+template <int NT, class F>
+__device__ __forceinline__ void oct_walk(const CellInfo* __restrict__ lc, const uint32_t* __restrict__ cand, int ncl,
+                                         const int* cpre, const int* tab, int T, F f) {
+  constexpr int U = kOctWalkChunk;
+  for (int kb = threadIdx.x; kb < T; kb += U * NT) {
+    uint32_t v[U];
+#pragma unroll
+    for (int u = 0; u < U; u++) {
+      const int k = kb + u * NT;
+      v[u] = 0;
+      if (k < T) {
+        int lo = 0, hi = ncl - 1;
+        while (lo < hi) {
+          const int mid = (lo + hi + 1) >> 1;
+          if (cpre[mid] <= k) lo = mid; else hi = mid - 1;
+        }
+        const int i = k - cpre[lo];
+        int off, ovf, kin;
+        if (tab) {
+          off = tab[lo];
+          ovf = tab[ncl + lo];
+          kin = tab[2 * ncl + lo];
+        } else {
+          const CellInfo& ci = lc[lo];
+          kin = ci.kin;
+          off = ci.cand_off;
+          ovf = ci.ovf_off - kin;
+        }
+        v[u] = cand[(i < kin ? off : ovf) + i];
+      }
+    }
+#pragma unroll
+    for (int u = 0; u < U; u++)
+      if (kb + u * NT < T) f(kb + u * NT, v[u]);
+  }
+}
+
 template <int NT>
 __device__ int oct_generic(const Geometry* __restrict__ G, const CellInfo* __restrict__ cells, const BatchPtrs& B,
                            const OctGroup& grp, unsigned char* smem_raw, int img, int l) {
@@ -988,7 +1044,9 @@
   int n_p1 = 0, n_p2 = 0;
 #endif
   const int ncl = L.cell_end - L.cell_begin;
-  for (int c = tid; c < ncl; c += NT) s.cpre[c] = B.cell_count[(size_t)img * G->ncells + L.cell_begin + c];
+  const CellInfo* lc = cells + L.cell_begin;
+  int* ctab = oct_cell_table_fits(ncl, NC) ? (int*)smem_raw : nullptr;
+  oct_stage_cells<NT>(lc, B.cell_count + (size_t)img * G->ncells + L.cell_begin, ncl, s.cpre, ctab);
   __syncthreads();
   const int T = block_exclusive_scan<NT>(s.cpre, ncl);
   if (tid == 0) s.cpre[ncl] = T;
@@ -1010,32 +1068,7 @@
     oc.set(k, pos, (uint32_t)root);
     atomicAdd(&s.ccnt[root], 1);
   };
-  if (ncl >= NT / 2) {
-    for (int c = tid; c < ncl; c += NT) {
-      const int k0 = s.cpre[c], n = s.cpre[c + 1] - k0;
-      const CellInfo& ci = cells[L.cell_begin + c];
-      const int kin = ci.kin, off = ci.cand_off, ovf = ci.ovf_off - kin;
-      int i = 0;
-      for (; i + 4 <= n; i += 4) {
-        const uint32_t v0 = cand[(i < kin ? off : ovf) + i], v1 = cand[(i + 1 < kin ? off : ovf) + i + 1],
-                       v2 = cand[(i + 2 < kin ? off : ovf) + i + 2], v3 = cand[(i + 3 < kin ? off : ovf) + i + 3];
-        put_cand(k0 + i, v0);
-        put_cand(k0 + i + 1, v1);
-        put_cand(k0 + i + 2, v2);
-        put_cand(k0 + i + 3, v3);
-      }
-      for (; i < n; i++) put_cand(k0 + i, cand[(i < kin ? off : ovf) + i]);
-    }
-  } else {
-    for (int k = tid; k < T; k += NT) {
-      int lo = 0, hi = ncl - 1;
-      while (lo < hi) {
-        const int mid = (lo + hi + 1) >> 1;
-        if (s.cpre[mid] <= k) lo = mid; else hi = mid - 1;
-      }
-      put_cand(k, cand[cell_slot(cells[L.cell_begin + lo], k - s.cpre[lo])]);
-    }
-  }
+  oct_walk<NT>(lc, cand, ncl, s.cpre, ctab, T, put_cand);
   __syncthreads();
   OCT_TS(ot1);
   for (int i = tid; i < nIni; i += NT) s.sa[i] = s.ccnt[i] > 0 ? 1 : 0;
@@ -1296,38 +1329,6 @@
   return 2;
 }
 
-template <int NT, class F>
-__device__ __forceinline__ void oct_walk(const LevelGeom& L, const CellInfo* __restrict__ cells,
-                                         const uint32_t* __restrict__ cand, const int* cpre, int T, F f) {
-  const int tid = threadIdx.x, ncl = L.cell_end - L.cell_begin;
-  if (ncl >= NT / 2) {
-    for (int c = tid; c < ncl; c += NT) {
-      const int k0 = cpre[c], n = cpre[c + 1] - k0;
-      const CellInfo& ci = cells[L.cell_begin + c];
-      const int kin = ci.kin, off = ci.cand_off, ovf = ci.ovf_off - kin;
-      int i = 0;
-      for (; i + 4 <= n; i += 4) {
-        const uint32_t v0 = cand[(i < kin ? off : ovf) + i], v1 = cand[(i + 1 < kin ? off : ovf) + i + 1],
-                       v2 = cand[(i + 2 < kin ? off : ovf) + i + 2], v3 = cand[(i + 3 < kin ? off : ovf) + i + 3];
-        f(k0 + i, v0);
-        f(k0 + i + 1, v1);
-        f(k0 + i + 2, v2);
-        f(k0 + i + 3, v3);
-      }
-      for (; i < n; i++) f(k0 + i, cand[(i < kin ? off : ovf) + i]);
-    }
-  } else {
-    for (int k = tid; k < T; k += NT) {
-      int lo = 0, hi = ncl - 1;
-      while (lo < hi) {
-        const int mid = (lo + hi + 1) >> 1;
-        if (cpre[mid] <= k) lo = mid; else hi = mid - 1;
-      }
-      f(k, cand[cell_slot(cells[L.cell_begin + lo], k - cpre[lo])]);
-    }
-  }
-}
-
 template <int NT>
 __device__ int oct_pyramid(const Geometry* __restrict__ G, const CellInfo* __restrict__ cells, const BatchPtrs& B,
                            const OctGroup& grp, int D, unsigned char* smem_raw, int img, int l) {
@@ -1359,7 +1360,9 @@
   int n_p1 = 0, n_p2 = 0;
 #endif
   const int ncl = L.cell_end - L.cell_begin;
-  for (int c = tid; c < ncl; c += NT) cpre[c] = B.cell_count[(size_t)img * G->ncells + L.cell_begin + c];
+  const CellInfo* lc = cells + L.cell_begin;
+  int* ctab = oct_cell_table_fits(ncl, NC) ? (int*)(smem_raw + lay.cnt) : nullptr;
+  oct_stage_cells<NT>(lc, B.cell_count + (size_t)img * G->ncells + L.cell_begin, ncl, cpre, ctab);
   __syncthreads();
   const int T = block_exclusive_scan<NT>(cpre, ncl);
   if (tid == 0) cpre[ncl] = T;
@@ -1405,7 +1408,7 @@
     gy = ytab[min(max(yr, 0), boxH - 1)];
   };
   const int kcap = grp.pcap;
-  oct_walk<NT>(L, cells, cand, cpre, T, [&](int k, uint32_t v) {
+  oct_walk<NT>(lc, cand, ncl, cpre, ctab, T, [&](int k, uint32_t v) {
     int gx, gy;
     leaf(v, gx, gy);
     const int idx = offD + gy * (nIni << D) + gx;
@@ -1626,6 +1629,7 @@
     key[i] = 0;
     pyr[slot((cell + cur * NC)[i])] = (uint16_t)i;
   }
+  if (T > grp.pcap) oct_stage_cells<NT>(lc, nullptr, ncl, nullptr, ctab);
   __syncthreads();
   auto hand_over = [&](int k, uint32_t v) {
     int gx, gy;
@@ -1643,7 +1647,7 @@
   if (T <= kcap) {
     for (int k = tid; k < T; k += NT) hand_over(k, kp[k]);
   } else {
-    oct_walk<NT>(L, cells, cand, cpre, T, hand_over);
+    oct_walk<NT>(lc, cand, ncl, cpre, ctab, T, hand_over);
   }
   __syncthreads();
   const int nout = min(S, L.oct_cap);
diff --git a/orb_slam2_commit_amd/csrc/orbx_extractor.h b/orb_slam2_commit_amd/csrc/orbx_extractor.h
--- a/orb_slam2_commit_amd/csrc/orbx_extractor.h
+++ b/orb_slam2_commit_amd/csrc/orbx_extractor.h
@@ -76,7 +76,6 @@
   orbx::DevBuf<uint8_t> in, out;
   size_t out_kps = 0, out_desc = 0, out_bytes = 0;
   orbx::PinnedBuf hstage;
-  orbx::DevBuf<uint64_t> rkeys;
   orbx::DevBuf<int2> rxi;
   orbx::DevBuf<uint4> rdesc;
   orbx::DevBuf<uint32_t> rtab;
diff --git a/orb_slam2_commit_amd/csrc/orbx_stereo.h b/orb_slam2_commit_amd/csrc/orbx_stereo.h
--- a/orb_slam2_commit_amd/csrc/orbx_stereo.h
+++ b/orb_slam2_commit_amd/csrc/orbx_stereo.h
@@ -26,7 +26,6 @@
   float* depth;
   int* sad;
   long long out_stride;
-  uint64_t* rkeys;
   int* oct_start;
   int2* rxi;
   uint4* rdesc;
@@ -39,6 +38,8 @@
 struct StageTimer;
 hipError_t launch_stereo(const StereoArgs& A, const Geometry* Gd, int n_frames, int maxL, hipStream_t st,
                          StageTimer* T);
+hipError_t launch_stereo_prep(const StereoArgs& A, const Geometry* Gd, int n_frames, hipStream_t st);
+hipError_t launch_stereo_finalize(const StereoArgs& A, int n_frames, hipStream_t st);
 hipError_t launch_hamming(const uint8_t* a, const uint8_t* b, int n, int32_t* out, hipStream_t st);
 
 }
diff --git a/orb_slam2_commit_amd/csrc/stereo.hip b/orb_slam2_commit_amd/csrc/stereo.hip
--- a/orb_slam2_commit_amd/csrc/stereo.hip
+++ b/orb_slam2_commit_amd/csrc/stereo.hip
@@ -13,43 +13,121 @@
 __device__ __forceinline__ uint32_t fbits(float f) { return __float_as_uint(f); }
 
 constexpr int PBS = 1024;
+constexpr int kSortBins = 6144;
+constexpr int kSortBinCap = 32;
+constexpr int kPrepKeys = kMaxStereoKps / PBS;
+
+__device__ __forceinline__ void prep_scan_excl(int* a, int n, int* wsum) {
+  const int tid = threadIdx.x, lane = tid & 63, wid = tid >> 6;
+  const int chunk = (n + PBS - 1) / PBS;
+  const int b = min(n, tid * chunk), e = min(n, b + chunk);
+  int local = 0;
+  for (int i = b; i < e; i++) local += a[i];
+  int incl = local;
+#pragma unroll
+  for (int o = 1; o < 64; o <<= 1) {
+    const int v = __shfl_up(incl, o, 64);
+    if (lane >= o) incl += v;
+  }
+  if (lane == 63) wsum[wid] = incl;
+  __syncthreads();
+  int run = incl - local;
+#pragma unroll
+  for (int w = 0; w < PBS / 64; w++) run += w < wid ? wsum[w] : 0;
+  for (int i = b; i < e; i++) {
+    const int v = a[i];
+    a[i] = run;
+    run += v;
+  }
+  __syncthreads();
+}
+
 __global__ __launch_bounds__(PBS) void k_stereo_prep(StereoArgs A, const Geometry* __restrict__ G) {
   __shared__ uint64_t keys[kMaxStereoKps];
+  __shared__ int bins[kSortBins];
+  __shared__ int wsum[PBS / 64];
   __shared__ int ost[kMaxLevelsPlan + 1];
   const int f = blockIdx.x, tid = threadIdx.x;
   const int nR = min(A.nR[(size_t)f * A.n_stride_R], kMaxStereoKps);
   const orbx_keypoint* kR = A.kpR + (size_t)f * A.kR_stride;
-  int P2 = 2;
-  while (P2 < nR) P2 <<= 1;
-  for (int i = tid; i < P2; i += PBS) {
-    uint64_t k = ~0ull;
+  const int nb = A.nlevels * A.rows;
+  const bool fits = nb <= kSortBins;
+  const uint32_t ylim = fbits((float)A.rows);
+  uint64_t key[kPrepKeys];
+  int bin[kPrepKeys], slot[kPrepKeys];
+  bool ok = fits;
+#pragma unroll
+  for (int j = 0; j < kPrepKeys; j++) {
+    const int i = tid + j * PBS;
+    key[j] = ~0ull;
+    bin[j] = -1;
+    slot[j] = 0;
     if (i < nR) {
-      const orbx_keypoint kp = kR[i];
-      k = ((uint64_t)(uint32_t)kp.octave << 44) | ((uint64_t)fbits(kp.y) << 12) | (uint64_t)i;
-    }
-    keys[i] = k;
-  }
-  __syncthreads();
-  for (int size = 2; size <= P2; size <<= 1) {
-    for (int stride = size >> 1; stride > 0; stride >>= 1) {
-      for (int i = tid; i < P2 / 2; i += PBS) {
-        const int lo = 2 * i - (i & (stride - 1));
-        const int hi = lo + stride;
-        const bool asc = (lo & size) == 0;
-        const uint64_t a = keys[lo], b = keys[hi];
-        if (asc ? (a > b) : (a < b)) {
-          keys[lo] = b;
-          keys[hi] = a;
+      const int o = kR[i].octave;
+      const float y = kR[i].y;
+      key[j] = ((uint64_t)(uint32_t)o << 44) | ((uint64_t)fbits(y) << 12) | (uint64_t)i;
+      if ((uint32_t)o < (uint32_t)A.nlevels && fbits(y) < ylim)
+        bin[j] = o * A.rows + (int)y;
+      else
+        ok = false;
+    }
+  }
+  if (fits)
+    for (int e = tid; e < nb; e += PBS) bins[e] = 0;
+  ok = !__syncthreads_or(!ok);
+  if (ok) {
+#pragma unroll
+    for (int j = 0; j < kPrepKeys; j++)
+      if (bin[j] >= 0) {
+        slot[j] = atomicAdd(&bins[bin[j]], 1);
+        if (slot[j] >= kSortBinCap) ok = false;
+      }
+    ok = !__syncthreads_or(!ok);
+  }
+  if (ok) {
+    prep_scan_excl(bins, nb, wsum);
+#pragma unroll
+    for (int j = 0; j < kPrepKeys; j++)
+      if (bin[j] >= 0) keys[bins[bin[j]] + slot[j]] = key[j];
+    __syncthreads();
+#pragma unroll
+    for (int j = 0; j < kPrepKeys; j++)
+      if (bin[j] >= 0 && slot[j] == 1) {
+        const int b = bins[bin[j]], e = bin[j] + 1 < nb ? bins[bin[j] + 1] : nR;
+        for (int a = b + 1; a < e; a++) {
+          const uint64_t v = keys[a];
+          int c = a;
+          for (; c > b && keys[c - 1] > v; c--) keys[c] = keys[c - 1];
+          keys[c] = v;
         }
       }
-      __syncthreads();
-    }
-  }
-  uint64_t* out = A.rkeys + (size_t)f * kMaxStereoKps;
+    __syncthreads();
+  } else {
+    int P2 = 2;
+    while (P2 < nR) P2 <<= 1;
+#pragma unroll
+    for (int j = 0; j < kPrepKeys; j++)
+      if (tid + j * PBS < P2) keys[tid + j * PBS] = key[j];
+    __syncthreads();
+    for (int size = 2; size <= P2; size <<= 1) {
+      for (int stride = size >> 1; stride > 0; stride >>= 1) {
+        for (int i = tid; i < P2 / 2; i += PBS) {
+          const int lo = 2 * i - (i & (stride - 1));
+          const int hi = lo + stride;
+          const bool asc = (lo & size) == 0;
+          const uint64_t a = keys[lo], b = keys[hi];
+          if (asc ? (a > b) : (a < b)) {
+            keys[lo] = b;
+            keys[hi] = a;
+          }
+        }
+        __syncthreads();
+      }
+    }
+  }
   int2* rxi = A.rxi + (size_t)f * kMaxStereoKps;
   for (int i = tid; i < nR; i += PBS) {
     const uint64_t k = keys[i];
-    out[i] = k;
     const int idx = (int)(k & 0xFFF);
     rxi[i] = make_int2(__float_as_int(kR[idx].x), idx);
   }
@@ -302,33 +380,71 @@
   }
 }
 
+struct BinSel {
+  int n, bin, rem;
+};
+__device__ __forceinline__ BinSel bin_select(const int* hist, int lane, int k) {
+  const int4 h = *reinterpret_cast<const int4*>(hist + 4 * lane);
+  const int s = h.x + h.y + h.z + h.w;
+  int incl = s;
+#pragma unroll
+  for (int o = 1; o < 64; o <<= 1) {
+    const int v = __shfl_up(incl, o, 64);
+    if (lane >= o) incl += v;
+  }
+  BinSel r;
+  r.n = __shfl(incl, 63, 64);
+  if (k < 0) k = r.n / 2;
+  const uint64_t m = __ballot(incl > k);
+  if (m == 0) {
+    r.bin = 256;
+    r.rem = k - r.n;
+    return r;
+  }
+  int acc = incl - s, j = 0;
+  if (acc + h.x <= k) {
+    acc += h.x;
+    j = 1;
+    if (acc + h.y <= k) {
+      acc += h.y;
+      j = 2;
+      if (acc + h.z <= k) {
+        acc += h.z;
+        j = 3;
+      }
+    }
+  }
+  const int owner = __builtin_ctzll(m);
+  r.bin = __shfl(4 * lane + j, owner, 64);
+  r.rem = __shfl(k - acc, owner, 64);
+  return r;
+}
+
 __global__ __launch_bounds__(SBS) void k_stereo_finalize(StereoArgs A) {
-  __shared__ int hist[256];
+  __shared__ __attribute__((aligned(16))) int hist[2][256];
   __shared__ int sel[4];
   const int f = blockIdx.x, tid = threadIdx.x;
   const int nL = min(A.nL[(size_t)f * A.n_stride_L], A.maxL);
   const int* sad = A.sad + (size_t)f * A.out_stride;
   float* uR = A.uR + (size_t)f * A.out_stride;
   float* depth = A.depth + (size_t)f * A.out_stride;
-  for (int i = tid; i < 256; i += SBS) hist[i] = 0;
+  for (int i = tid; i < 256; i += SBS) {
+    hist[0][i] = 0;
+    hist[1][i] = 0;
+  }
   __syncthreads();
   for (int i = tid; i < nL; i += SBS) {
     const int s = sad[i];
-    if (s >= 0) atomicAdd(&hist[(s >> 8) & 255], 1);
-  }
-  __syncthreads();
-  if (tid == 0) {
-    int n = 0;
-    for (int b = 0; b < 256; b++) n += hist[b];
-    sel[0] = n;
-    const int k = n / 2;
-    int acc = 0, b = 0;
-    for (; b < 256; b++) {
-      if (acc + hist[b] > k) break;
-      acc += hist[b];
-    }
-    sel[1] = b;
-    sel[2] = k - acc;
+    if (s >= 0) atomicAdd(&hist[0][(s >> 8) & 255], 1);
+  }
+  __syncthreads();
+  if (tid < 64) {
+    const BinSel r = bin_select(hist[0], tid, -1);
+    if (tid == 0) {
+      sel[0] = r.n;
+      sel[1] = r.bin;
+      sel[2] = r.rem;
+    }
   }
   __syncthreads();
   const int n = sel[0];
@@ -337,21 +453,14 @@
     return;
   }
   const int hb = sel[1], k2 = sel[2];
-  __syncthreads();
-  for (int i = tid; i < 256; i += SBS) hist[i] = 0;
-  __syncthreads();
   for (int i = tid; i < nL; i += SBS) {
     const int s = sad[i];
-    if (s >= 0 && ((s >> 8) & 255) == hb) atomicAdd(&hist[s & 255], 1);
-  }
-  __syncthreads();
-  if (tid == 0) {
-    int acc = 0, b = 0;
-    for (; b < 256; b++) {
-      if (acc + hist[b] > k2) break;
-      acc += hist[b];
-    }
-    sel[3] = (hb << 8) | b;
+    if (s >= 0 && ((s >> 8) & 255) == hb) atomicAdd(&hist[1][s & 255], 1);
+  }
+  __syncthreads();
+  if (tid < 64) {
+    const BinSel r = bin_select(hist[1], tid, k2);
+    if (tid == 0) sel[3] = (hb << 8) | r.bin;
   }
   __syncthreads();
   const float median = (float)sel[3];
@@ -483,6 +592,16 @@
   return hipGetLastError();
 }
 
+hipError_t launch_stereo_prep(const StereoArgs& A, const Geometry* Gd, int n_frames, hipStream_t st) {
+  hipLaunchKernelGGL(k_stereo_prep, dim3(n_frames), dim3(PBS), 0, st, A, Gd);
+  return hipGetLastError();
+}
+
+hipError_t launch_stereo_finalize(const StereoArgs& A, int n_frames, hipStream_t st) {
+  hipLaunchKernelGGL(k_stereo_finalize, dim3(n_frames), dim3(SBS), 0, st, A);
+  return hipGetLastError();
+}
+
 hipError_t launch_hamming(const uint8_t* a, const uint8_t* b, int n, int32_t* out, hipStream_t st) {
   if (n <= 0) return hipSuccess;
   hipLaunchKernelGGL(k_hamming, dim3((n + SBS - 1) / SBS), dim3(SBS), 0, st, a, b, n, out);
diff --git a/orb_slam2_commit_amd/orb.py b/orb_slam2_commit_amd/orb.py
--- a/orb_slam2_commit_amd/orb.py
+++ b/orb_slam2_commit_amd/orb.py
@@ -157,6 +157,29 @@
                                                  ptr(depth), ptr(sad), ptr(nm)),
           "orbx_debug_stereo_keypoints")
     return uR, depth, sad, int(nm[0])
+
+
+def debug_stereo_prep(extractor, kps_right):
+    kR = np.ascontiguousarray(kps_right, KEYPOINT_DTYPE)
+    nR = len(kR)
+    h = extractor._last_shape[1]
+    order = np.zeros(nR, np.int32)
+    oct_start = np.zeros(extractor.nlevels + 1, np.int32)
+    rtab = np.zeros((extractor.nlevels, h), np.uint32)
+    check(_lib.lib().orbx_debug_stereo_prep(extractor._h, ptr(kR), nR, ptr(order), ptr(oct_start), ptr(rtab)),
+          "orbx_debug_stereo_prep")
+    return order, oct_start, rtab
+
+
+def debug_stereo_median(sad, u_right, depth, device=0):
+    s = np.ascontiguousarray(sad, np.int32)
+    uR = np.array(u_right, np.float32)
+    dep = np.array(depth, np.float32)
+    assert uR.shape == s.shape == dep.shape
+    nm = np.zeros(1, np.int32)
+    check(_lib.lib().orbx_debug_stereo_median(ptr(s), len(s), ptr(uR), ptr(dep), ptr(nm), int(device)),
+          "orbx_debug_stereo_median")
+    return uR, dep, int(nm[0])
 
 
 def debug_launch_plan(params, width, height, what, a0=0, a1=0, a2=0):
```

New measurement: 120,800 frames/s (median of 6 runs). Within noise of the previous version (+0.4%).
